# google-research/seed_rl

Hardware: NVIDIA H100
Metric: env-frames/sec (learner, device-timed) on synthetic 84x84x4 T=20 unrolls @1/2/4/8 H100 (higher is better)
Workload: dtype bf16x3 (fp32-faithful tensor-core contraction; activations stored as bf16 hi+lo pairs), f32 elsewhere

## Files before the change

include/seedrl_b200.h:

```cpp
#ifndef SEEDRL_B200_H_
#define SEEDRL_B200_H_

#include <stddef.h>
#include <stdint.h>

#ifdef __cplusplus
extern "C" {
#endif

#define SEEDRL_OK 0
#define SEEDRL_ERR_INVALID_ARGUMENT 3
#define SEEDRL_ERR_OUT_OF_RANGE 11
#define SEEDRL_ERR_INTERNAL 13
#define SEEDRL_ERR_CANCELLED 1
#define SEEDRL_ERR_UNAVAILABLE 14

typedef void* seedrl_stream_t;

const char* seedrl_last_error(void);
int seedrl_abi_version(void);
uint64_t seedrl_kernel_launch_count(void);

int seedrl_vtrace_from_importance_weights(
    int T, int B,
    const float* target_action_log_probs, const float* behaviour_action_log_probs,
    const float* discounts, const float* rewards, const float* values,
    const float* bootstrap_value,
    float clip_rho_threshold, float clip_pg_rho_threshold, float lambda_,
    float* vs, float* pg_advantages, seedrl_stream_t stream);

int seedrl_categorical_log_prob(int N, int A, const float* logits,
                                const int64_t* actions, float* log_prob,
                                seedrl_stream_t stream);
int seedrl_categorical_entropy(int N, int A, const float* logits, float* entropy,
                               seedrl_stream_t stream);
int seedrl_categorical_sample(int N, int A, const float* logits,
                              const float* gumbel_noise, uint64_t seed,
                              uint64_t offset, int64_t* actions,
                              seedrl_stream_t stream);
int seedrl_categorical_sample_counter(int N, int A, const float* logits, const float* gumbel_noise,
                                      uint64_t seed, uint64_t* counter_dev, int64_t* actions,
                                      seedrl_stream_t stream);

typedef struct seedrl_loss_config {
  float discounting;
  float lambda_;
  float baseline_cost;
  float kl_cost;
  float max_abs_reward;
  float clip_rho_threshold;
  float clip_pg_rho_threshold;
  float target_entropy;
  int32_t has_target_entropy;
  float entropy_cost_adjustment_speed;
} seedrl_loss_config;

enum {
  SEEDRL_LT_TOTAL = 0, SEEDRL_LT_POLICY = 1, SEEDRL_LT_V = 2, SEEDRL_LT_ENTROPY = 3,
  SEEDRL_LT_KL = 4, SEEDRL_LT_ENTROPY_ADJ = 5, SEEDRL_LT_V_MEAN = 6,
  SEEDRL_LT_V_L2_ERROR = 7, SEEDRL_LT_MEAN_ENTROPY = 8, SEEDRL_LT_ENTROPY_COST = 9,
  SEEDRL_LT_MEAN_KL = 10, SEEDRL_LT_MAX_ACTION_ABS = 11,
  SEEDRL_LOSS_TERMS = 16
};

size_t seedrl_vtrace_loss_scratch_bytes(int T1, int B, int A);
int seedrl_vtrace_loss_fwd_bwd(
    int T1, int B, int A,
    const float* learner_logits, const float* learner_baseline,
    const float* behaviour_logits, const int64_t* actions,
    const float* rewards, const uint8_t* done,
    const seedrl_loss_config* cfg, const float* entropy_cost_param,
    float* loss_terms, float* dlogits, float* dbaseline,
    float* d_entropy_cost_param, float* vs_out, float* pg_advantages_out,
    void* scratch, seedrl_stream_t stream);

int seedrl_adam_apply(size_t n, float* params, const float* grads, float* m,
                      float* v, float lr_t, float beta1, float beta2, float eps,
                      float grad_scale, int64_t clamp_index, float clamp_lo,
                      float clamp_hi, seedrl_stream_t stream);

enum { SEEDRL_NET_DEEP = 0, SEEDRL_NET_SHALLOW = 1 };

typedef struct seedrl_net_config {
  int32_t net;
  int32_t num_actions;
  int32_t obs_h, obs_w, obs_c;
} seedrl_net_config;

typedef struct seedrl_net seedrl_net;

int seedrl_net_create(const seedrl_net_config* cfg, seedrl_net** out);
void seedrl_net_destroy(seedrl_net* net);
int seedrl_net_num_param_tensors(const seedrl_net* net);
size_t seedrl_net_num_params(const seedrl_net* net);
size_t seedrl_net_arena_floats(const seedrl_net* net);
int seedrl_net_set_conv_mode(seedrl_net* net, int mode);
int seedrl_net_set_lstm_mode(seedrl_net* net, int mode);
int seedrl_net_param_info(const seedrl_net* net, int index, char* name_buf,
                          size_t name_buf_len, int64_t* dims, size_t* offset);
size_t seedrl_net_workspace_bytes(const seedrl_net* net, int T1, int B);

int seedrl_net_forward(const seedrl_net* net, const float* params, int T1, int B,
                       const int64_t* prev_actions, const float* reward,
                       const uint8_t* done, const uint8_t* observation,
                       const float* h0, const float* c0,
                       float* policy_logits, float* baseline,
                       float* h_out, float* c_out,
                       void* workspace, size_t workspace_bytes,
                       seedrl_stream_t stream);
int seedrl_net_backward(const seedrl_net* net, const float* params, int T1, int B,
                        const int64_t* prev_actions, const float* reward,
                        const uint8_t* done, const uint8_t* observation,
                        const float* dlogits, const float* dbaseline,
                        float* grads, void* workspace, size_t workspace_bytes,
                        seedrl_stream_t stream);
int seedrl_net_backward_overlap(const seedrl_net* net, const float* params, int T1, int B,
                                const int64_t* prev_actions, const float* reward, const uint8_t* done,
                                const uint8_t* observation, const float* dlogits, const float* dbaseline,
                                float* grads, void* workspace, size_t workspace_bytes,
                                void* head_ready_event, seedrl_stream_t stream);
size_t seedrl_net_grad_split(const seedrl_net* net);
int seedrl_net_check_error(const seedrl_net* net, int T1, int B, void* workspace,
                           size_t workspace_bytes, seedrl_stream_t stream);

int seedrl_store_append_field(uint8_t* state, const int32_t* index,
                              const int32_t* env_ids, int n, int full_length,
                              size_t row_bytes, const uint8_t* values,
                              seedrl_stream_t stream);
int seedrl_store_advance(int32_t* index, const int32_t* env_ids, int n,
                         int full_length, int32_t* completed_ids,
                         int32_t* num_completed, seedrl_stream_t stream);
int seedrl_store_advance_limit(int32_t* index, const int32_t* env_ids, int n,
                               int full_length, int32_t* completed_ids,
                               int32_t* num_completed, int32_t id_limit,
                               seedrl_stream_t stream);
int seedrl_store_gather_field(uint8_t* state, const int32_t* completed_ids,
                              int n_completed, int full_length, size_t row_bytes,
                              int overlap, int time_major, uint8_t* unrolls,
                              seedrl_stream_t stream);
#define SEEDRL_MAX_ROW_JOBS 16
typedef struct seedrl_row_job {
  void* table;
  void* rows;
  size_t row_bytes;
  int32_t mode;
  int32_t full_length;
} seedrl_row_job;
int seedrl_rows_multi(const seedrl_row_job* jobs, int njobs, const int32_t* env_ids, int n,
                      const int32_t* index, seedrl_stream_t stream);
int seedrl_rows_multi_limit(const seedrl_row_job* jobs, int njobs, const int32_t* env_ids, int n,
                            const int32_t* index, int32_t id_limit, seedrl_stream_t stream);
int seedrl_store_gather_field_into(uint8_t* state, const int32_t* completed_ids, int n_completed,
                                   int full_length, size_t row_bytes, int overlap, uint8_t* batch,
                                   int batch_cols, int col0, seedrl_stream_t stream);
int seedrl_store_finish(int32_t* index, const int32_t* completed_ids,
                        int n_completed, int overlap, seedrl_stream_t stream);
int seedrl_store_reset(uint8_t* state, int32_t* index, const int32_t* env_ids,
                       int n, int full_length, size_t row_bytes, int overlap,
                       seedrl_stream_t stream);

typedef struct seedrl_batcher seedrl_batcher;
int seedrl_batcher_create(int batch_size, int num_slabs, int n_in,
                          const size_t* in_row_bytes, int n_out,
                          const size_t* out_row_bytes, int pinned,
                          seedrl_batcher** out);
void seedrl_batcher_destroy(seedrl_batcher* b);
int seedrl_batcher_claim(seedrl_batcher* b, int k, int* slab, int* row);
void* seedrl_batcher_input_ptr(seedrl_batcher* b, int slab, int field, int row);
void* seedrl_batcher_output_ptr(seedrl_batcher* b, int slab, int field, int row);
int seedrl_batcher_commit(seedrl_batcher* b, int slab, int k);
int seedrl_batcher_wait_outputs(seedrl_batcher* b, int slab, int* status);
int seedrl_batcher_release(seedrl_batcher* b, int slab);
int seedrl_batcher_next_full(seedrl_batcher* b, int timeout_ms, int* slab);
int seedrl_batcher_publish(seedrl_batcher* b, int slab, int status);
int seedrl_batcher_shutdown(seedrl_batcher* b);

int seedrl_profile_num_categories(void);
const char* seedrl_profile_category_name(int i);
int seedrl_profile_begin(seedrl_stream_t stream);
int seedrl_profile_end(double* ms_per_category, uint64_t* launches_per_category);

typedef struct seedrl_r2d2_net seedrl_r2d2_net;
int seedrl_r2d2_net_create(int num_actions, int obs_h, int obs_w, int channels, seedrl_r2d2_net** out);
void seedrl_r2d2_net_destroy(seedrl_r2d2_net* net);
int seedrl_r2d2_net_num_param_tensors(const seedrl_r2d2_net* net);
size_t seedrl_r2d2_net_num_params(const seedrl_r2d2_net* net);
size_t seedrl_r2d2_net_arena_floats(const seedrl_r2d2_net* net);
int seedrl_r2d2_net_set_mode(seedrl_r2d2_net* net, int mode);
int seedrl_r2d2_net_set_lstm_mode(seedrl_r2d2_net* net, int mode);
int seedrl_r2d2_net_param_info(const seedrl_r2d2_net* net, int index, char* name_buf, size_t name_buf_len,
                               int64_t* dims4, int* rank, size_t* offset_floats);
size_t seedrl_r2d2_net_workspace_bytes(const seedrl_r2d2_net* net, int T, int B);
int seedrl_r2d2_net_forward(const seedrl_r2d2_net* net, const float* params, int T, int B,
                            const int64_t* prev_actions, const float* reward, const uint8_t* done,
                            const uint8_t* frames, const float* h0, const float* c0, float* q_values,
                            int32_t* action, float* h_out, float* c_out, void* workspace,
                            size_t workspace_bytes, seedrl_stream_t stream);
int seedrl_r2d2_net_backward(const seedrl_r2d2_net* net, const float* params, int T, int B,
                             const uint8_t* frames, const uint8_t* done, const float* dq, float* grads,
                             void* workspace, size_t workspace_bytes, seedrl_stream_t stream);
int seedrl_r2d2_net_check_error(const seedrl_r2d2_net* net, int T, int B, void* workspace,
                                size_t workspace_bytes, seedrl_stream_t stream);

int seedrl_r2d2_stack_frames(int T, int B, int P, int stack_size, const uint8_t* frames,
                             const int32_t* state_in, const uint8_t* done, uint8_t* stacked,
                             int32_t* state_out, seedrl_stream_t stream);
size_t seedrl_r2d2_loss_scratch_bytes(int T, int B, int n_steps);
int seedrl_r2d2_loss_fwd_bwd(int T, int B, int A, const float* q_train, const float* q_target,
                             const int64_t* replay_action, const float* reward, const uint8_t* done,
                             const float* importance_weights, float gamma, int n_steps, float eta,
                             float value_rescaling_eps, float* loss, float* priorities, float* dq,
                             void* scratch, seedrl_stream_t stream);
int seedrl_r2d2_epsilon_greedy(int N, int A, const int32_t* env_ids, const float* envs_epsilon,
                               uint64_t seed, uint64_t* counter_dev, int32_t* actions,
                               seedrl_stream_t stream);
int seedrl_replay_sample(int limit, const float* priorities, float priority_exp,
                         float importance_sampling_exp, int num_samples, const float* uniforms,
                         int64_t* indices, float* weights, float* probs_out, seedrl_stream_t stream);
size_t seedrl_clip_scratch_bytes(void);
int seedrl_clip_by_global_norm(size_t n, float* grads, float clip_norm, float* norm_out,
                               void* scratch, seedrl_stream_t stream);

int seedrl_debug_conv3x3(int cin, int cout, int in_mode, int N, int H, int W,
                         const void* in, const float* w, const float* bias,
                         const float* mask, const float* res, float* out,
                         seedrl_stream_t stream);
int seedrl_debug_conv3x3_flip(int cin, int cout, const float* w, float* wt,
                              seedrl_stream_t stream);
size_t seedrl_debug_wgrad_partial_bytes(void);
int seedrl_debug_conv_pixels(int N, int H, int W, int which, int start, int count, int* out);
int seedrl_debug_set_loss_stream(int enabled);
int seedrl_debug_set_wgrad_chunk(int kc);
int seedrl_debug_set_conv_tile(int mt);
int seedrl_debug_set_gemm_bk(int bk);
int seedrl_debug_set_gemm_gather(int on);
int seedrl_debug_set_first_layer_dense(int on);
int seedrl_debug_conv0pool(int N, int H, int W, const uint8_t* frames, const float* w, const float* bias,
                           void* praw, void* prelu, uint8_t* idx, int* err, seedrl_stream_t stream);
int seedrl_debug_conv0pool_c(int N, int H, int W, int C, const uint8_t* frames, const float* w, const float* bias,
                             void* praw, void* prelu, uint8_t* idx, int* err, seedrl_stream_t stream);
int seedrl_debug_first_wgrad_pooled_c(int N, int H, int W, int C, const uint8_t* frames, const void* g_planes,
                                      const uint8_t* idx, float* dw, float* db, float* partial,
                                      size_t partial_bytes, seedrl_stream_t stream);
int seedrl_debug_conv3x3_wgrad(int cin, int cout, int in_mode, int N, int H, int W,
                               const void* x, const float* dy, float* dw, float* db,
                               float* partial, size_t partial_bytes,
                               seedrl_stream_t stream);
int seedrl_debug_conv3x3_tc(int cin, int cout, int in_mode, int split, int N, int H, int W,
                            const void* in, const float* w, const float* bias,
                            const float* mask, const float* res, float* out, int flip,
                            int variant, void* wq_scratch, int* error_flag,
                            seedrl_stream_t stream);
int seedrl_debug_conv3x3_wgrad_tc(int cin, int cout, int in_mode, int split, int N, int H, int W,
                                  const void* x, const float* dy, float* dw, float* db,
                                  float* partial, size_t partial_bytes, int* error_flag,
                                  seedrl_stream_t stream);
int seedrl_debug_maxpool(int backward, int N, int H, int W, int C, const float* x_or_dy,
                         float* y_or_dx, uint8_t* idx, seedrl_stream_t stream);
int seedrl_debug_gemm_tc(int ta, int tb, int split, int M, int N, int K, const float* A, int lda,
                         const float* B, int ldb, float* C, int ldc, const float* bias,
                         const float* mask, int ldm, int relu, int accumulate, int a_relu,
                         float* ws, size_t ws_bytes, int* error_flag, seedrl_stream_t stream);
int seedrl_debug_colsum(int M, int N, const float* X, int ld, float* out, float* ws, size_t ws_bytes,
                        seedrl_stream_t stream);
int seedrl_debug_sgemm(int ta, int tb, int M, int N, int K, const float* A, int lda,
                       const float* B, int ldb, float* C, int ldc, const float* bias,
                       const float* mask, int ldm, int relu, int accumulate, int a_relu,
                       seedrl_stream_t stream);
int seedrl_debug_strided_conv(int op, int mode, int gather, int in_u8, int N, int H, int W, int C, int K,
                              int S, int cout, const void* x, const float* w, const float* bias,
                              const float* dy, const float* mask, float* out, int ldo, float* dbias,
                              float* col, size_t col_bytes, float* ws, size_t ws_bytes, int* error_flag,
                              int* gathered, seedrl_stream_t stream);
size_t seedrl_debug_lstm_workspace_bytes(int mode, int H, int T1, int B);
int seedrl_debug_lstm_forward(int mode, int gemm_mode, int H, int T1, int B, const float* U, const uint8_t* done,
                              float* z, const float* h0, const float* c0, float* hs, float* cs, float* hp,
                              void* ws, size_t ws_bytes, int* error_flag, seedrl_stream_t stream);
int seedrl_debug_lstm_backward(int mode, int gemm_mode, int H, int T1, int B, const float* U, const uint8_t* done,
                               const float* gates, const float* cs, const float* c0, const float* dhs, float* dz,
                               void* ws, size_t ws_bytes, int* error_flag, seedrl_stream_t stream);

size_t seedrl_debug_planes_bytes(int N, int H, int W, int C);
int seedrl_debug_to_planes(int N, int H, int W, int C, int relu, const float* x, void* out,
                           seedrl_stream_t stream);
int seedrl_debug_from_planes(int N, int H, int W, int C, const void* in, float* y,
                             seedrl_stream_t stream);
int seedrl_debug_convp(int cin, int cout, int N, int H, int W, const void* in, const float* w,
                       const float* bias, const void* mask, const void* res, int flip,
                       void* out_raw, void* out_relu, float* out_nhwc, void* wq_scratch,
                       int* error_flag, seedrl_stream_t stream);
int seedrl_debug_wgradp(int cin, int cout, int N, int H, int W, const void* x, const void* dy,
                        float* dw, float* db, float* partial, size_t partial_bytes,
                        int* error_flag, seedrl_stream_t stream);
int seedrl_debug_poolp(int backward, int N, int H, int W, int C, const void* in, void* out_raw,
                       void* out_relu, float* out_nhwc, uint8_t* idx, seedrl_stream_t stream);

#ifdef __cplusplus
}
#endif
#endif
```

seed_rl_b200/_lib.py:

```python
import ctypes
import os

_HERE = os.path.dirname(os.path.abspath(__file__))
LIB_PATH = os.path.join(_HERE, 'libseedrl_b200.so')

c_void_p, c_int, c_float, c_size_t = ctypes.c_void_p, ctypes.c_int, ctypes.c_float, ctypes.c_size_t
c_i64, c_u64 = ctypes.c_int64, ctypes.c_uint64
P = c_void_p


class SeedrlError(RuntimeError):

  def __init__(self, code, msg):
    super().__init__('libseedrl_b200 error %d: %s' % (code, msg))
    self.code = code


class LossConfig(ctypes.Structure):
  _fields_ = [('discounting', c_float), ('lambda_', c_float), ('baseline_cost', c_float),
              ('kl_cost', c_float), ('max_abs_reward', c_float),
              ('clip_rho_threshold', c_float), ('clip_pg_rho_threshold', c_float),
              ('target_entropy', c_float), ('has_target_entropy', ctypes.c_int32),
              ('entropy_cost_adjustment_speed', c_float)]


class RowJob(ctypes.Structure):
  _fields_ = [('table', ctypes.c_void_p), ('rows', ctypes.c_void_p), ('row_bytes', ctypes.c_size_t),
              ('mode', ctypes.c_int32), ('full_length', ctypes.c_int32)]


ROW_GATHER, ROW_SCATTER, ROW_APPEND = 0, 1, 2


def rows_multi(jobs, env_ids_i32, index=None, id_limit=None):
  n = int(env_ids_i32.numel())
  arr = (RowJob * len(jobs))()
  for k, (table, rows, mode) in enumerate(jobs):
    rb = (table[0, 0] if mode == ROW_APPEND else table[0]).numel() * table.element_size()
    if rows.numel() * rows.element_size() != n * rb or rows.dtype != table.dtype or not rows.is_contiguous():
      raise ValueError('rows_multi: rows do not match the table (job %d)' % k)
    arr[k] = RowJob(table.data_ptr(), rows.data_ptr(), rb, mode, table.shape[1] if mode == ROW_APPEND else 0)
  if id_limit is None:
    check(lib().seedrl_rows_multi(arr, len(jobs), ptr(env_ids_i32), n, ptr(index), stream_ptr()))
  else:
    check(lib().seedrl_rows_multi_limit(arr, len(jobs), ptr(env_ids_i32), n, ptr(index), int(id_limit),
                                        stream_ptr()))


class NetConfig(ctypes.Structure):
  _fields_ = [('net', ctypes.c_int32), ('num_actions', ctypes.c_int32),
              ('obs_h', ctypes.c_int32), ('obs_w', ctypes.c_int32), ('obs_c', ctypes.c_int32)]


NET_DEEP, NET_SHALLOW = 0, 1
LOSS_TERMS = 16
LT = dict(total=0, policy=1, V=2, entropy=3, kl=4, entropy_adj=5, v_mean=6, v_l2_error=7,
          mean_entropy=8, entropy_cost=9, mean_kl=10, max_action_abs=11)

SIGNATURES = {
    'seedrl_last_error': (ctypes.c_char_p, []),
    'seedrl_abi_version': (c_int, []),
    'seedrl_kernel_launch_count': (c_u64, []),
    'seedrl_vtrace_from_importance_weights':
        (c_int, [c_int, c_int, P, P, P, P, P, P, c_float, c_float, c_float, P, P, P]),
    'seedrl_categorical_log_prob': (c_int, [c_int, c_int, P, P, P, P]),
    'seedrl_categorical_entropy': (c_int, [c_int, c_int, P, P, P]),
    'seedrl_categorical_sample': (c_int, [c_int, c_int, P, P, c_u64, c_u64, P, P]),
    'seedrl_categorical_sample_counter': (c_int, [c_int, c_int, P, P, c_u64, P, P, P]),
    'seedrl_vtrace_loss_scratch_bytes': (c_size_t, [c_int, c_int, c_int]),
    'seedrl_vtrace_loss_fwd_bwd':
        (c_int, [c_int, c_int, c_int, P, P, P, P, P, P, ctypes.POINTER(LossConfig), P,
                 P, P, P, P, P, P, P, P]),
    'seedrl_adam_apply':
        (c_int, [c_size_t, P, P, P, P, c_float, c_float, c_float, c_float, c_float, c_i64,
                 c_float, c_float, P]),
    'seedrl_net_create': (c_int, [ctypes.POINTER(NetConfig), ctypes.POINTER(P)]),
    'seedrl_net_destroy': (None, [P]),
    'seedrl_net_num_param_tensors': (c_int, [P]),
    'seedrl_net_num_params': (c_size_t, [P]),
    'seedrl_net_arena_floats': (c_size_t, [P]),
    'seedrl_net_set_conv_mode': (c_int, [P, c_int]),
    'seedrl_net_set_lstm_mode': (c_int, [P, c_int]),
    'seedrl_net_param_info':
        (c_int, [P, c_int, ctypes.c_char_p, c_size_t, ctypes.POINTER(c_i64),
                 ctypes.POINTER(c_size_t)]),
    'seedrl_net_workspace_bytes': (c_size_t, [P, c_int, c_int]),
    'seedrl_net_forward':
        (c_int, [P, P, c_int, c_int, P, P, P, P, P, P, P, P, P, P, P, c_size_t, P]),
    'seedrl_net_backward':
        (c_int, [P, P, c_int, c_int, P, P, P, P, P, P, P, P, c_size_t, P]),
    'seedrl_net_backward_overlap':
        (c_int, [P, P, c_int, c_int, P, P, P, P, P, P, P, P, c_size_t, P, P]),
    'seedrl_net_grad_split': (c_size_t, [P]),
    'seedrl_net_check_error': (c_int, [P, c_int, c_int, P, c_size_t, P]),
    'seedrl_store_append_field': (c_int, [P, P, P, c_int, c_int, c_size_t, P, P]),
    'seedrl_store_advance': (c_int, [P, P, c_int, c_int, P, P, P]),
    'seedrl_store_advance_limit': (c_int, [P, P, c_int, c_int, P, P, ctypes.c_int32, P]),
    'seedrl_store_gather_field': (c_int, [P, P, c_int, c_int, c_size_t, c_int, c_int, P, P]),
    'seedrl_rows_multi': (c_int, [P, c_int, P, c_int, P, P]),
    'seedrl_rows_multi_limit': (c_int, [P, c_int, P, c_int, P, ctypes.c_int32, P]),
    'seedrl_store_gather_field_into': (c_int, [P, P, c_int, c_int, c_size_t, c_int, P, c_int, c_int, P]),
    'seedrl_store_finish': (c_int, [P, P, c_int, c_int, P]),
    'seedrl_store_reset': (c_int, [P, P, P, c_int, c_int, c_size_t, c_int, P]),
    'seedrl_batcher_create':
        (c_int, [c_int, c_int, c_int, ctypes.POINTER(c_size_t), c_int, ctypes.POINTER(c_size_t),
                 c_int, ctypes.POINTER(P)]),
    'seedrl_batcher_destroy': (None, [P]),
    'seedrl_batcher_claim': (c_int, [P, c_int, ctypes.POINTER(c_int), ctypes.POINTER(c_int)]),
    'seedrl_batcher_input_ptr': (P, [P, c_int, c_int, c_int]),
    'seedrl_batcher_output_ptr': (P, [P, c_int, c_int, c_int]),
    'seedrl_batcher_commit': (c_int, [P, c_int, c_int]),
    'seedrl_batcher_wait_outputs': (c_int, [P, c_int, ctypes.POINTER(c_int)]),
    'seedrl_batcher_release': (c_int, [P, c_int]),
    'seedrl_batcher_next_full': (c_int, [P, c_int, ctypes.POINTER(c_int)]),
    'seedrl_batcher_publish': (c_int, [P, c_int, c_int]),
    'seedrl_batcher_shutdown': (c_int, [P]),
    'seedrl_r2d2_net_create': (c_int, [c_int, c_int, c_int, c_int, ctypes.POINTER(P)]),
    'seedrl_r2d2_net_destroy': (None, [P]),
    'seedrl_r2d2_net_num_param_tensors': (c_int, [P]),
    'seedrl_r2d2_net_num_params': (c_size_t, [P]),
    'seedrl_r2d2_net_arena_floats': (c_size_t, [P]),
    'seedrl_r2d2_net_set_mode': (c_int, [P, c_int]),
    'seedrl_r2d2_net_set_lstm_mode': (c_int, [P, c_int]),
    'seedrl_r2d2_net_param_info':
        (c_int, [P, c_int, ctypes.c_char_p, c_size_t, ctypes.POINTER(c_i64), ctypes.POINTER(c_int),
                 ctypes.POINTER(c_size_t)]),
    'seedrl_r2d2_net_workspace_bytes': (c_size_t, [P, c_int, c_int]),
    'seedrl_r2d2_net_forward':
        (c_int, [P, P, c_int, c_int, P, P, P, P, P, P, P, P, P, P, P, c_size_t, P]),
    'seedrl_r2d2_net_backward': (c_int, [P, P, c_int, c_int, P, P, P, P, P, c_size_t, P]),
    'seedrl_r2d2_net_check_error': (c_int, [P, c_int, c_int, P, c_size_t, P]),
    'seedrl_r2d2_stack_frames': (c_int, [c_int, c_int, c_int, c_int, P, P, P, P, P, P]),
    'seedrl_r2d2_loss_scratch_bytes': (c_size_t, [c_int, c_int, c_int]),
    'seedrl_r2d2_loss_fwd_bwd': (c_int, [c_int, c_int, c_int, P, P, P, P, P, P, c_float, c_int, c_float, c_float,
                                         P, P, P, P, P]),
    'seedrl_r2d2_epsilon_greedy': (c_int, [c_int, c_int, P, P, c_u64, P, P, P]),
    'seedrl_replay_sample': (c_int, [c_int, P, c_float, c_float, c_int, P, P, P, P, P]),
    'seedrl_clip_scratch_bytes': (c_size_t, []),
    'seedrl_clip_by_global_norm': (c_int, [c_size_t, P, c_float, P, P, P]),
    'seedrl_profile_num_categories': (c_int, []),
    'seedrl_profile_category_name': (ctypes.c_char_p, [c_int]),
    'seedrl_profile_begin': (c_int, [P]),
    'seedrl_profile_end': (c_int, [ctypes.POINTER(ctypes.c_double), ctypes.POINTER(c_u64)]),
    'seedrl_debug_planes_bytes': (c_size_t, [c_int, c_int, c_int, c_int]),
    'seedrl_debug_to_planes': (c_int, [c_int, c_int, c_int, c_int, c_int, P, P, P]),
    'seedrl_debug_from_planes': (c_int, [c_int, c_int, c_int, c_int, P, P, P]),
    'seedrl_debug_convp': (c_int, [c_int, c_int, c_int, c_int, c_int, P, P, P, P, P, c_int, P, P, P, P, P, P]),
    'seedrl_debug_wgradp': (c_int, [c_int, c_int, c_int, c_int, c_int, P, P, P, P, P, c_size_t, P, P]),
    'seedrl_debug_poolp': (c_int, [c_int, c_int, c_int, c_int, c_int, P, P, P, P, P, P]),
    'seedrl_debug_conv3x3': (c_int, [c_int, c_int, c_int, c_int, c_int, c_int, P, P, P, P, P, P, P]),
    'seedrl_debug_conv3x3_flip': (c_int, [c_int, c_int, P, P, P]),
    'seedrl_debug_conv3x3_tc':
        (c_int, [c_int, c_int, c_int, c_int, c_int, c_int, c_int, P, P, P, P, P, P, c_int, c_int, P, P, P]),
    'seedrl_debug_wgrad_partial_bytes': (c_size_t, []),
    'seedrl_debug_conv_pixels': (c_int, [c_int, c_int, c_int, c_int, c_int, c_int, P]),
    'seedrl_debug_set_loss_stream': (c_int, [c_int]),
    'seedrl_debug_set_wgrad_chunk': (c_int, [c_int]),
    'seedrl_debug_set_conv_tile': (c_int, [c_int]),
    'seedrl_debug_set_gemm_bk': (c_int, [c_int]),
    'seedrl_debug_set_first_layer_dense': (c_int, [c_int]),
    'seedrl_debug_conv0pool': (c_int, [c_int, c_int, c_int, P, P, P, P, P, P, P, P]),
    'seedrl_debug_conv0pool_c': (c_int, [c_int, c_int, c_int, c_int, P, P, P, P, P, P, P, P]),
    'seedrl_debug_first_wgrad_pooled_c': (c_int, [c_int, c_int, c_int, c_int, P, P, P, P, P, P, c_size_t, P]),
    'seedrl_debug_conv3x3_wgrad_tc':
        (c_int, [c_int, c_int, c_int, c_int, c_int, c_int, c_int, P, P, P, P, P, c_size_t, P, P]),
    'seedrl_debug_conv3x3_wgrad':
        (c_int, [c_int, c_int, c_int, c_int, c_int, c_int, P, P, P, P, P, c_size_t, P]),
    'seedrl_debug_maxpool': (c_int, [c_int, c_int, c_int, c_int, c_int, P, P, P, P]),
    'seedrl_debug_gemm_tc':
        (c_int, [c_int, c_int, c_int, c_int, c_int, c_int, P, c_int, P, c_int, P, c_int, P, P, c_int, c_int, c_int,
                 c_int, P, c_size_t, P, P]),
    'seedrl_debug_set_gemm_gather': (c_int, [c_int]),
    'seedrl_debug_colsum': (c_int, [c_int, c_int, P, c_int, P, P, c_size_t, P]),
    'seedrl_debug_sgemm':
        (c_int, [c_int, c_int, c_int, c_int, c_int, P, c_int, P, c_int, P, c_int, P, P, c_int,
                 c_int, c_int, c_int, P]),
    'seedrl_debug_strided_conv':
        (c_int, [c_int, c_int, c_int, c_int, c_int, c_int, c_int, c_int, c_int, c_int, c_int, P, P, P, P, P, P,
                 c_int, P, P, c_size_t, P, c_size_t, P, ctypes.POINTER(c_int), P]),
    'seedrl_debug_lstm_workspace_bytes': (c_size_t, [c_int, c_int, c_int, c_int]),
    'seedrl_debug_lstm_forward':
        (c_int, [c_int, c_int, c_int, c_int, c_int, P, P, P, P, P, P, P, P, P, c_size_t, P, P]),
    'seedrl_debug_lstm_backward':
        (c_int, [c_int, c_int, c_int, c_int, c_int, P, P, P, P, P, P, P, P, c_size_t, P, P]),
}

_lib = None


def lib():
  global _lib
  if _lib is None:
    if not os.path.exists(LIB_PATH):
      raise ImportError(
          'seed_rl_b200: %s is missing -- build it with `python -c "import '
          '__graft_entry__ as g; g.build()"` (seed_rl_b200/csrc/build.sh). There is no '
          'CPU or PyTorch fallback.' % LIB_PATH)
    l = ctypes.CDLL(LIB_PATH)
    for name, (res, args) in SIGNATURES.items():
      fn = getattr(l, name)
      fn.restype = res
      fn.argtypes = args
    _lib = l
  return _lib


def check(rc):
  if rc != 0:
    raise SeedrlError(rc, (lib().seedrl_last_error() or b'').decode('utf-8', 'replace'))


def launch_count():
  return int(lib().seedrl_kernel_launch_count())


def ptr(t):
  return None if t is None else ctypes.c_void_p(t.data_ptr())


def stream_ptr():
  import torch
  return ctypes.c_void_p(torch.cuda.current_stream().cuda_stream)


def require_cuda(t, dtype, name):
  import torch
  if not isinstance(t, torch.Tensor):
    t = torch.as_tensor(t)
  if not torch.cuda.is_available():
    raise RuntimeError('seed_rl_b200 needs a CUDA device (H100); there is no CPU path '
                       '(argument %r).' % name)
  if t.device.type != 'cuda':
    t = t.cuda()
  if t.dtype != dtype:
    t = t.to(dtype)
  return t.contiguous()
```

seed_rl_b200/common/inference_host.py:

```python
from absl import logging
import numpy as np
import torch

from seed_rl_b200 import _lib
from seed_rl_b200.common import utils
from seed_rl_b200.grpc import ops as grpc


class InferenceHostBase(object):

  algorithm = None

  def __init__(self, agent, num_envs, inference_batch_size, observation_shape, action_dtype,
               agent_state_specs, agent_output_specs, unroll_length, num_overlapping_steps=0,
               time_major=False, id_limit=None, num_action_repeats=1, device='cuda', info_queue=None,
               use_graph=False):
    self.agent = agent
    self.device = torch.device(device)
    self.N = N = int(inference_batch_size)
    self.num_action_repeats = num_action_repeats
    TS = utils.TensorSpec
    self.env_output_specs = utils.EnvOutput(
        TS([], 'float32', 'reward'), TS([], 'bool', 'done'), TS(list(observation_shape), 'uint8', 'observation'),
        TS([], 'bool', 'abandoned'), TS([], 'int32', 'episode_step'))
    action_specs = TS([], action_dtype, 'action')
    self.agent_state_specs = agent_state_specs
    self._id_limit = id_limit
    self._num_store_envs = num_envs if id_limit is None else id_limit
    self.store = utils.UnrollStore(self._num_store_envs, unroll_length,
                                   (action_specs, self.env_output_specs, agent_output_specs),
                                   num_overlapping_steps=num_overlapping_steps, device=device, time_major=time_major)
    self.env_run_ids = np.zeros([num_envs], np.int64)
    self.env_infos = [np.zeros([num_envs], np.int64), np.zeros([num_envs], np.float32),
                      np.zeros([num_envs], np.float32)]
    self.first_agent_states = utils.Aggregator(num_envs, agent_state_specs, 'first_agent_states', device)
    self.agent_states = utils.Aggregator(num_envs, agent_state_specs, 'agent_states', device)
    self.actions = utils.Aggregator(num_envs, action_specs, 'actions', device)
    self.info_queue = info_queue
    self.inference_specs = (
        TS([N], 'int32', 'env_id'), TS([N], 'int64', 'run_id'),
        utils.map_structure(lambda s: TS([N] + list(s.shape), s.dtype, s.name), self.env_output_specs),
        TS([N], 'float32', 'raw_reward'))
    self.output_specs = TS([N], action_dtype, 'action')
    self.stream = torch.cuda.Stream(device=self.device)
    self.use_graph = bool(use_graph)
    if self.use_graph and not 1 <= N <= num_envs:
      raise ValueError('cuda_graph needs 1 <= inference_batch_size <= num_envs, got %d and %d' % (N, num_envs))
    self._graph = None
    self._actions_pin = torch.zeros([N], dtype=utils.as_torch_dtype(action_dtype)).pin_memory()

    @grpc.function(self.inference_specs, self.output_specs)
    def inference(env_ids, run_ids, env_outputs, raw_rewards):
      return self._inference(env_ids, run_ids, env_outputs, raw_rewards)
    self.inference = inference

  def _policy(self, ids32, prev_actions, env_outputs, prev_states, counter):
    raise NotImplementedError

  def _completed_unrolls(self, nc):
    raise NotImplementedError

  def _episode_infos(self, done_ids):
    return tuple(torch.as_tensor(t[done_ids]) for t in self.env_infos)

  def _begin_batch(self, env_ids, run_ids, env_outputs, raw_rewards):
    if np.asarray(env_outputs.abandoned).any():
      raise ValueError('Abandoned done states are not supported in %s.' % self.algorithm)
    utils._check_no_duplicates(None, env_ids, 'inference batch')
    previous = self.env_run_ids[env_ids]
    self.env_run_ids[env_ids] = run_ids
    reset_ids = env_ids[previous != run_ids]
    if reset_ids.size:
      logging.info('Environment ids needing reset: %s', reset_ids)
      for t in self.env_infos:
        t[reset_ids] = 0
      self.store.reset(reset_ids[reset_ids < self._num_store_envs])
      init = self.agent.initial_state(len(reset_ids))
      self.first_agent_states.replace(reset_ids, init)
      self.agent_states.replace(reset_ids, init)
      self.actions.reset(reset_ids)
    self.env_infos[1][env_ids] += np.asarray(env_outputs.reward)
    self.env_infos[2][env_ids] += np.asarray(raw_rewards)
    done_ids = env_ids[np.asarray(env_outputs.done)]
    if self.info_queue is not None and done_ids.size:
      self.info_queue.enqueue_many(self._episode_infos(done_ids))
    for t in self.env_infos:
      t[done_ids] = 0
    self.env_infos[0][env_ids] += self.num_action_repeats

  def _device_step(self, ids32, env_dev, counter):
    n = int(ids32.numel())
    tables = self.agent_states._state
    prev_actions = torch.empty([n], dtype=self.actions._state[0].dtype, device=self.device)
    prev_states = [torch.empty([n] + list(t.shape[1:]), dtype=t.dtype, device=self.device) for t in tables]
    _lib.rows_multi([(self.actions._state[0], prev_actions, _lib.ROW_GATHER)] +
                    [(t, r, _lib.ROW_GATHER) for t, r in zip(tables, prev_states)], ids32)
    agent_outputs, curr_states = self._policy(
        ids32, prev_actions, env_dev, utils.pack_sequence_as(self.agent_state_specs, prev_states), counter)
    self.store.device_append(ids32, utils.flatten((prev_actions, env_dev, agent_outputs)), id_limit=self._id_limit)
    _lib.rows_multi([(t, r.contiguous(), _lib.ROW_SCATTER) for t, r in zip(tables, utils.flatten(curr_states))] +
                    [(self.actions._state[0], agent_outputs.action.contiguous(), _lib.ROW_SCATTER)], ids32)
    return prev_states, agent_outputs

  def _build_graph(self):
    N, dev = self.N, self.device
    self._g_ids = torch.arange(N, dtype=torch.int32, device=dev)
    self._g_env = utils.EnvOutput(*(torch.zeros([N] + list(s.shape), dtype=utils.as_torch_dtype(s.dtype), device=dev)
                                    for s in self.env_output_specs))
    self._g_pin = [torch.zeros_like(t, device='cpu').pin_memory() for t in (self._g_ids,) + tuple(self._g_env)]
    self._g_counter = torch.zeros([], dtype=torch.int64, device=dev)
    touched = (self.actions._state + self.agent_states._state + self.store._state +
               [self.store._index, self._g_counter])
    saved = [t.clone() for t in touched]
    self._device_step(self._g_ids, self._g_env, self._g_counter)
    for t, sv in zip(touched, saved):
      t.copy_(sv)
    self.stream.synchronize()
    g = torch.cuda.CUDAGraph()
    with torch.cuda.graph(g, stream=self.stream, capture_error_mode='thread_local'):
      self._g_prev_states, self._g_out = self._device_step(self._g_ids, self._g_env, self._g_counter)
    self._graph = g

  def _inference(self, env_ids, run_ids, env_outputs, raw_rewards):
    env_ids, run_ids = np.asarray(env_ids), np.asarray(run_ids)
    n = len(env_ids)
    with torch.cuda.stream(self.stream):
      self._begin_batch(env_ids, run_ids, env_outputs, raw_rewards)
      if self.use_graph and n == self.N:
        if self._graph is None:
          self._build_graph()
        srcs = (env_ids.astype(np.int32),) + tuple(np.asarray(x) for x in env_outputs)
        for pin, dst, src in zip(self._g_pin, (self._g_ids,) + tuple(self._g_env), srcs):
          t = torch.from_numpy(np.ascontiguousarray(src))
          if t.numel() >= 65536 and t.is_pinned():
            dst.copy_(t, non_blocking=True)
          else:
            pin.numpy()[...] = src
            dst.copy_(pin, non_blocking=True)
        self._graph.replay()
        prev_states, agent_outputs = self._g_prev_states, self._g_out
      else:
        ids32 = torch.as_tensor(env_ids.astype(np.int32)).to(self.device, non_blocking=True)
        env_dev = utils.EnvOutput(*(torch.as_tensor(np.asarray(x)).to(self.device, non_blocking=True)
                                    for x in env_outputs))
        prev_states, agent_outputs = self._device_step(ids32, env_dev, None)
      store_pos = np.nonzero(env_ids < self._num_store_envs)[0]
      done_ids, pos = self.store.host_advance(env_ids[store_pos])
      pending = None
      if done_ids.size:
        completed_ids, pending = self._completed_unrolls(int(done_ids.size))
        pos_dev = torch.as_tensor(store_pos[pos].astype(np.int64)).to(self.device, non_blocking=True)
        self.first_agent_states.replace(completed_ids, [t.index_select(0, pos_dev) for t in prev_states],
                                        check_unique=False)
      actions = self._actions_pin[:n]
      actions.copy_(agent_outputs.action, non_blocking=True)
      self.stream.synchronize()
    if pending is not None:
      self.unroll_queue.enqueue_many(pending)
    return actions.numpy().copy()
```

seed_rl_b200/csrc/conv_planes.cu:

```cuda
#include <cuda.h>
#include <cuda_bf16.h>

#include <cstdio>
#include <cstdlib>

#include "kernels.h"
#include "tc_common.cuh"

namespace seedrl {

long long planes_positions(int N, int H, int W) {
  const long long Q = (long long)N * (H + 1) * (W + 2);
  return ((Q + 2 * (W + 2) + 2 + 256 + 127) / 128) * 128;
}
size_t planes_bytes(int N, int H, int W, int C) {
  return (size_t)planes_positions(N, H, W) * 16 * 2 * (C / 8);
}

typedef CUresult (*EncodeTiledFn)(CUtensorMap*, CUtensorMapDataType, cuuint32_t, void*, const cuuint64_t*,
                                  const cuuint64_t*, const cuuint32_t*, const cuuint32_t*,
                                  CUtensorMapInterleave, CUtensorMapSwizzle, CUtensorMapL2promotion,
                                  CUtensorMapFloatOOBfill);
static EncodeTiledFn encode_tiled_fn() {
  static EncodeTiledFn fn = nullptr;
  static bool tried = false;
  if (!tried) {
    tried = true;
    void* q = nullptr;
    cudaDriverEntryPointQueryResult qr;
    if (cudaGetDriverEntryPoint("cuTensorMapEncodeTiled", &q, cudaEnableDefault, &qr) == cudaSuccess &&
        qr == cudaDriverEntryPointSuccess)
      fn = reinterpret_cast<EncodeTiledFn>(q);
    (void)cudaGetLastError();
  }
  return fn;
}

static int g_chunk = 0;
int planes_chunk() {
  if (g_chunk == 0) {
    const char* e = getenv("SEEDRL_PLANES_CHUNK");
    g_chunk = e ? atoi(e) : 128;
    if (g_chunk != 16 && g_chunk != 32 && g_chunk != 64 && g_chunk != 128) g_chunk = 128;
  }
  return g_chunk;
}

static int make_plane_map(CUtensorMap* tm, const void* base, long long Lp, int planes, int shift,
                          int CH, int box_chunks, int box_planes) {
  EncodeTiledFn enc = encode_tiled_fn();
  if (!enc) return set_error(SEEDRL_ERR_INTERNAL, "cuTensorMapEncodeTiled is not available");
  if (box_chunks < 1 || box_chunks > 256 || box_planes < 1 || box_planes > planes)
    return set_error(SEEDRL_ERR_INVALID_ARGUMENT, "conv planes: TMA box out of range");
  const cuuint64_t gdim[3] = {(cuuint64_t)(2 * CH), (cuuint64_t)((Lp - shift) / CH), (cuuint64_t)planes};
  const cuuint64_t gstr[2] = {(cuuint64_t)CH * 16, (cuuint64_t)Lp * 16};
  const cuuint32_t box[3] = {(cuuint32_t)(2 * CH), (cuuint32_t)box_chunks, (cuuint32_t)box_planes};
  const cuuint32_t estr[3] = {1, 1, 1};
  void* addr = const_cast<char*>(reinterpret_cast<const char*>(base)) + (size_t)shift * 16;
  const CUresult r = enc(tm, CU_TENSOR_MAP_DATA_TYPE_UINT64, 3, addr, gdim, gstr, box, estr,
                         CU_TENSOR_MAP_INTERLEAVE_NONE, CU_TENSOR_MAP_SWIZZLE_NONE,
                         CU_TENSOR_MAP_L2_PROMOTION_L2_256B, CU_TENSOR_MAP_FLOAT_OOB_FILL_NONE);
  if (r != CUDA_SUCCESS) {
    char msg[128];
    snprintf(msg, sizeof msg, "cuTensorMapEncodeTiled failed (%d) Lp=%lld planes=%d shift=%d box=%dx%d", (int)r, Lp,
             planes, shift, box_chunks, box_planes);
    return set_error(SEEDRL_ERR_INTERNAL, msg);
  }
  return SEEDRL_OK;
}

__device__ __forceinline__ void mbar_expect_tx(uint64_t* bar, uint32_t bytes) {
  asm volatile("mbarrier.arrive.expect_tx.shared::cta.b64 _, [%0], %1;" ::"r"(smem_u32(bar)), "r"(bytes)
               : "memory");
}
__device__ __forceinline__ void tma_load_3d(void* dst, const CUtensorMap* tm, int c0, int c1, int c2,
                                            uint64_t* bar) {
  asm volatile(
      "cp.async.bulk.tensor.3d.shared::cluster.global.tile.mbarrier::complete_tx::bytes [%0], [%1, {%2, %3, %4}], [%5];" ::
          "r"(smem_u32(dst)),
      "l"(reinterpret_cast<uint64_t>(tm)), "r"(c0), "r"(c1), "r"(c2), "r"(smem_u32(bar))
      : "memory");
}
__device__ __forceinline__ float bf16lo(uint32_t w) { return __uint_as_float(w << 16); }
__device__ __forceinline__ float bf16hi(uint32_t w) { return __uint_as_float(w & 0xFFFF0000u); }

struct ConvpArgs {
  ConvGeom g;
  int Lp;
  int nch;
  int chunk;
  int ntiles;
  int nb;
  const uint4* wq;
  const float* bias;
  const uint4* mask;
  const uint4* res;
  uint4* out_raw;
  uint4* out_relu;
  float* out_nhwc;
  int* err;
};

constexpr int kCpWarpgroups = 4;
constexpr int kCpThreads = 128 * kCpWarpgroups + 32;
constexpr int kCpM = 128;
constexpr int kCpMaxStages = 4;

__device__ __forceinline__ void quad_transpose(float2 (&t)[4], int q) {
#pragma unroll
  for (int b = 1; b <= 2; b <<= 1) {
    const bool up = (q & b) != 0;
#pragma unroll
    for (int u = 0; u < 4; ++u) {
      if (u & b) continue;
      const float2 send = up ? t[u] : t[u | b];
      const float2 r = make_float2(__shfl_xor_sync(0xffffffffu, send.x, b), __shfl_xor_sync(0xffffffffu, send.y, b));
      if (up) t[u] = r; else t[u | b] = r;
    }
  }
}

template <int CIN, int COUT, int NSUB>
__global__ void __launch_bounds__(kCpThreads, 1)
convp_kernel(const __grid_constant__ CUtensorMap tm_in, const ConvpArgs a) {
  constexpr int G = CIN / 8, GO = COUT / 8, NS = CIN / 16;
  constexpr int MT = NSUB * kCpM;
  constexpr int NBLK = 2 * NSUB;
  extern __shared__ __align__(128) uint8_t smem_raw[];
  const int PW = a.g.PW, nb = a.nb;
  const uint32_t P = (uint32_t)(a.nch * a.chunk) * 16u;
  const uint32_t stage_bytes = 2u * G * P;
  uint8_t* s_stage = smem_raw;
  uint4* s_b = reinterpret_cast<uint4*>(smem_raw + (size_t)nb * stage_bytes);
  float* s_bias = reinterpret_cast<float*>(s_b + 2 * 9 * CIN * COUT / 8);
  uint64_t* s_full = reinterpret_cast<uint64_t*>(s_bias + COUT);
  uint64_t* s_empty = s_full + kCpMaxStages;
  const int tid = threadIdx.x, warp = tid >> 5, lane = tid & 31;

  for (int i = tid; i < 2 * 9 * CIN * COUT / 8; i += kCpThreads) s_b[i] = __ldg(a.wq + i);
  if (tid < COUT) s_bias[tid] = a.bias ? __ldg(a.bias + tid) : 0.f;
  if (tid == 0) {
    for (int i = 0; i < nb; ++i) {
      mbar_init(s_full + i, 1);
      mbar_init(s_empty + i, 4 * kCpWarpgroups);
    }
    asm volatile("fence.mbarrier_init.release.cluster;" ::: "memory");
    asm volatile("prefetch.tensormap [%0];" ::"l"(reinterpret_cast<uint64_t>(&tm_in)) : "memory");
  }
  asm volatile("fence.proxy.async.shared::cta;" ::: "memory");
  __syncthreads();

  const int my_tiles = ((int)blockIdx.x < a.ntiles) ? (a.ntiles - 1 - (int)blockIdx.x) / (int)gridDim.x + 1 : 0;
  bool timed_out = false;

  if (warp == 4 * kCpWarpgroups) {
    if (elect_one()) {
      for (int it = 0; it < my_tiles; ++it) {
        const int s = it % nb;
        if (it >= nb && !mbar_wait_bounded(s_empty + s, (uint32_t)(((it / nb) - 1) & 1))) { timed_out = true; break; }
        const int tile = (int)blockIdx.x + it * (int)gridDim.x;
        mbar_expect_tx(s_full + s, stage_bytes);
        tma_load_3d(s_stage + (size_t)s * stage_bytes, &tm_in, 0, tile * MT / a.chunk, 0, s_full + s);
      }
    }
    __syncwarp();
  } else {
    const int cw = warp >> 2;
    const size_t plane_u = (size_t)a.Lp;
    if (blockIdx.x == 0) {
      const uint4 z = make_uint4(0u, 0u, 0u, 0u);
      for (int i = tid; i < (PW + 1) * 2 * GO; i += 128 * kCpWarpgroups) {
        const int pl = i / (PW + 1), s = i - pl * (PW + 1);
        if (a.out_raw) a.out_raw[(size_t)pl * plane_u + s] = z;
        if (a.out_relu) a.out_relu[(size_t)pl * plane_u + s] = z;
      }
    }
    const int q = lane & 3;
    const int row = 16 * (warp & 3) + (lane >> 2) + 8 * (q & 1);
    const uint32_t b_base = smem_u32(s_b);
    const uint64_t db0 = gmma_desc(b_base, (uint32_t)(2 * GO) * 128u, 128u);
    for (int it = 0; it < my_tiles; ++it) {
      const int s = it % nb;
      const int tile = (int)blockIdx.x + it * (int)gridDim.x;
      if (!mbar_wait_bounded(s_full + s, (uint32_t)((it / nb) & 1))) { timed_out = true; break; }
      const int m0 = (cw - it * NBLK) & (kCpWarpgroups - 1);
      if (m0 >= NBLK && lane == 0) mbar_arrive(s_empty + s);
      const uint32_t a_base = smem_u32(s_stage + (size_t)s * stage_bytes);
      const uint64_t da0 = gmma_desc(a_base, P, 128u);
      const uint64_t lo_off = (uint64_t)((G * P) >> 4), slab_off = (uint64_t)((2 * P) >> 4);
#pragma unroll 1
      for (int m = m0; m < NBLK; m += kCpWarpgroups) {
        float acc[COUT];
#pragma unroll
        for (int i = 0; i < COUT; ++i) acc[i] = 0.f;
        wgmma_fence_acc<COUT>(acc);
        wgmma_fence();
#pragma unroll
        for (int tap = 0; tap < 9; ++tap) {
          const uint64_t off = (uint64_t)(m * 64 + (tap / 3) * PW + (tap % 3));
#pragma unroll
          for (int sl = 0; sl < NS; ++sl) {
            const uint64_t da = da0 + off + (uint64_t)sl * slab_off;
            const uint64_t db = db0 + (uint64_t)((tap * NS + sl) * (COUT * 64 / 16));
            Wgmma<2 * COUT>::template mma<0, 0>(acc, da, db, 1u);
            Wgmma<COUT>::template mma<0, 0>(acc, da + lo_off, db, 1u);
          }
        }
        wgmma_commit();
        const int p = tile * MT + m * 64 + row;
        const int sp = p + PW + 1;
        const int pix = out_pixel(a.g, p);
        uint4 mk[GO / 2], rh[GO / 2], rl[GO / 2];
        if (pix >= 0) {
#pragma unroll
          for (int k = 0; k < GO / 2; ++k) {
            const int go = (q >> 1) + 2 * k;
            if (a.mask) mk[k] = __ldg(a.mask + (size_t)go * plane_u + sp);
            if (a.res) {
              rh[k] = __ldg(a.res + (size_t)go * plane_u + sp);
              rl[k] = __ldg(a.res + (size_t)(GO + go) * plane_u + sp);
            }
          }
        }
        wgmma_wait<0>();
        wgmma_fence_acc<COUT>(acc);
        if (m + kCpWarpgroups >= NBLK && lane == 0) mbar_arrive(s_empty + s);
        const bool in_store = sp < a.Lp;
#pragma unroll
        for (int k = 0; k < GO / 2; ++k) {
          const int go = (q >> 1) + 2 * k;
          float2 t[4];
#pragma unroll
          for (int u = 0; u < 4; ++u) {
            const int j = 2 * k + (u >> 1), h = u & 1;
            t[u] = make_float2(acc[4 * j + 2 * h] + acc[4 * (j + GO) + 2 * h],
                               acc[4 * j + 2 * h + 1] + acc[4 * (j + GO) + 2 * h + 1]);
          }
          quad_transpose(t, q);
          float x[8];
#pragma unroll
          for (int e = 0; e < 4; ++e) {
            x[2 * e] = t[e].x + s_bias[go * 8 + 2 * e];
            x[2 * e + 1] = t[e].y + s_bias[go * 8 + 2 * e + 1];
          }
          if (pix >= 0 && a.mask) {
            const uint32_t mw[4] = {mk[k].x, mk[k].y, mk[k].z, mk[k].w};
#pragma unroll
            for (int e = 0; e < 4; ++e) {
              x[2 * e] = bf16lo(mw[e]) > 0.f ? x[2 * e] : 0.f;
              x[2 * e + 1] = bf16hi(mw[e]) > 0.f ? x[2 * e + 1] : 0.f;
            }
          }
          if (pix >= 0 && a.res) {
            const uint32_t hw[4] = {rh[k].x, rh[k].y, rh[k].z, rh[k].w};
            const uint32_t lw[4] = {rl[k].x, rl[k].y, rl[k].z, rl[k].w};
#pragma unroll
            for (int e = 0; e < 4; ++e) {
              x[2 * e] += bf16lo(hw[e]) + bf16lo(lw[e]);
              x[2 * e + 1] += bf16hi(hw[e]) + bf16hi(lw[e]);
            }
          }
          if (pix < 0) {
#pragma unroll
            for (int e = 0; e < 8; ++e) x[e] = 0.f;
          }
          const float4 xa = make_float4(x[0], x[1], x[2], x[3]), xb = make_float4(x[4], x[5], x[6], x[7]);
          if (a.out_raw && in_store) {
            a.out_raw[(size_t)go * plane_u + sp] = pack8_bf16(xa, xb);
            a.out_raw[(size_t)(GO + go) * plane_u + sp] = pack8_bf16(bf16_resid4(xa), bf16_resid4(xb));
          }
          if (a.out_relu && in_store) {
            const float4 ra = make_float4(fmaxf(xa.x, 0.f), fmaxf(xa.y, 0.f), fmaxf(xa.z, 0.f), fmaxf(xa.w, 0.f));
            const float4 rb = make_float4(fmaxf(xb.x, 0.f), fmaxf(xb.y, 0.f), fmaxf(xb.z, 0.f), fmaxf(xb.w, 0.f));
            a.out_relu[(size_t)go * plane_u + sp] = pack8_bf16(ra, rb);
            a.out_relu[(size_t)(GO + go) * plane_u + sp] = pack8_bf16(bf16_resid4(ra), bf16_resid4(rb));
          }
          if (a.out_nhwc && pix >= 0) {
            float4* o = reinterpret_cast<float4*>(a.out_nhwc + (size_t)pix * COUT + go * 8);
            o[0] = xa; o[1] = xb;
          }
        }
      }
    }
  }
  if (timed_out && a.err) atomicExch(a.err, 1);
}

template <int CIN, int COUT, int NSUB>
static int launch_convp(const PlaneConv& c, cudaStream_t st) {
  const ConvGeom g = make_geom(c.N, c.H, c.W);
  constexpr int MT = NSUB * kCpM;
  const long long Lp = planes_positions(c.N, c.H, c.W);
  if (Lp + MT + 4 * g.PW >= (1LL << 31))
    return set_error(SEEDRL_ERR_INVALID_ARGUMENT, "convp: batch too large for 32-bit positions");
  const int L = MT + 2 * g.PW + 2;
  const int CH = planes_chunk();
  const int nch = (L + CH - 1) / CH;
  const size_t stage = (size_t)2 * (CIN / 8) * nch * CH * 16;
  const size_t fixed = (size_t)2 * 9 * CIN * COUT * 2 + COUT * 4 + 2 * kCpMaxStages * 8;
  int nb = kCpMaxStages;
  while (nb > 1 && nb * stage + fixed > 227 * 1024) --nb;
  if (nb < 2) return kPlanesTryNext;
  const size_t smem = nb * stage + fixed;
  CUtensorMap tm;
  SEEDRL_TRY(make_plane_map(&tm, c.in, Lp, 2 * (CIN / 8), 0, CH, nch, 2 * (CIN / 8)));
  static bool attr = false;
  if (!attr) {
    SEEDRL_CUDA(cudaFuncSetAttribute(convp_kernel<CIN, COUT, NSUB>, cudaFuncAttributeMaxDynamicSharedMemorySize,
                                     227 * 1024));
    attr = true;
  }
  ConvpArgs a;
  a.g = g; a.Lp = (int)Lp; a.nch = nch; a.chunk = CH; a.nb = nb;
  a.ntiles = (int)((Lp - g.PW - 1 + MT - 1) / MT);
  a.wq = reinterpret_cast<const uint4*>(c.wq); a.bias = c.bias;
  a.mask = reinterpret_cast<const uint4*>(c.mask); a.res = reinterpret_cast<const uint4*>(c.res);
  a.out_raw = reinterpret_cast<uint4*>(c.out_raw); a.out_relu = reinterpret_cast<uint4*>(c.out_relu);
  a.out_nhwc = c.out_nhwc; a.err = c.err;
  const int grid = a.ntiles < kNumSMs ? a.ntiles : kNumSMs;
  convp_kernel<CIN, COUT, NSUB><<<grid, kCpThreads, smem, st>>>(tm, a);
  count_launch(g_conv_cat, st);
  SEEDRL_CHECK_LAUNCH();
  return SEEDRL_OK;
}

bool convp_supported(int cin, int cout) {
  return (cin == 16 || cin == 32) && (cout == 16 || cout == 32);
}

int convp_forward(int cin, int cout, const PlaneConv& c, cudaStream_t st) {
  const long long Lp = planes_positions(c.N, c.H, c.W);
  const bool small = Lp / 512 < 2 * kNumSMs;
#define SEEDRL_CP_CASE(CI, CO_)                                                   \
  if (cin == CI && cout == CO_) {                                                 \
    int rc = kPlanesTryNext;                                                      \
    if (!small) rc = launch_convp<CI, CO_, 4>(c, st);                             \
    if (rc == kPlanesTryNext) rc = launch_convp<CI, CO_, 2>(c, st);               \
    if (rc == kPlanesTryNext) rc = launch_convp<CI, CO_, 1>(c, st);               \
    if (rc == kPlanesTryNext) return set_error(SEEDRL_ERR_INVALID_ARGUMENT, "convp: image too wide"); \
    return rc;                                                                    \
  }
  SEEDRL_CP_CASE(16, 16)
  SEEDRL_CP_CASE(16, 32)
  SEEDRL_CP_CASE(32, 16)
  SEEDRL_CP_CASE(32, 32)
#undef SEEDRL_CP_CASE
  return set_error(SEEDRL_ERR_INVALID_ARGUMENT, "convp: unsupported (cin,cout)");
}

struct WgradpArgs {
  int PW, T, nchunks, nb;
  int chunk;
  float* partial;
  int* err;
};

constexpr int kWpMaxStages = 6;
constexpr int kWpHaloRow = 8;
__host__ __device__ constexpr int wgradp_mtiles(int CP) { return 3 * CP + 1 <= 64 ? 1 : 2; }
__host__ __device__ constexpr int wgradp_khsplit(int CP) { return CP == 16 ? 3 : 1; }
__host__ __device__ constexpr int wgradp_threads(int CP) { return 128 * wgradp_mtiles(CP) * wgradp_khsplit(CP) + 32; }

struct WgradMaps { CUtensorMap x, x_halo, dy, dy_halo; };

template <int CP, int COUT, int KC>
__global__ void __launch_bounds__(wgradp_threads(CP), 1)
wgradp_kernel(const __grid_constant__ WgradMaps tm, const WgradpArgs a) {
  constexpr int G = CP / 8, GO = COUT / 8;
  constexpr int MT = wgradp_mtiles(CP), KSPL = wgradp_khsplit(CP), NCW = MT * KSPL;
  constexpr int NKH = 3 / KSPL;
  constexpr int NW = 9 * CP * COUT + COUT;
  constexpr uint32_t Px = (KC + kWpHaloRow) * 16;
  extern __shared__ __align__(128) uint8_t smem_raw[];
  const int nb = a.nb, PW = a.PW;
  const uint32_t Pd = (uint32_t)(KC + a.T) * 16u;
  const uint32_t x_bytes = 2u * G * Px;
  const uint32_t stage_bytes = x_bytes + 2u * GO * Pd;
  uint64_t* s_full = reinterpret_cast<uint64_t*>(smem_raw);
  uint64_t* s_empty = s_full + kWpMaxStages;
  uint8_t* s_stage = smem_raw + 128;
  const int tid = threadIdx.x, warp = tid >> 5, lane = tid & 31;

  if (tid == 0) {
    for (int i = 0; i < kWpMaxStages; ++i) { mbar_init(s_full + i, 1); mbar_init(s_empty + i, 4 * NCW); }
    asm volatile("fence.mbarrier_init.release.cluster;" ::: "memory");
  }
  __syncthreads();

  const int my_chunks = ((int)blockIdx.x < a.nchunks) ? (a.nchunks - 1 - (int)blockIdx.x) / (int)gridDim.x + 1 : 0;
  bool timed_out = false;

  if (warp == 4 * NCW) {
    if (elect_one()) {
      for (int it = 0; it < my_chunks; ++it) {
        const int s = it % nb;
        if (it >= nb && !mbar_wait_bounded(s_empty + s, (uint32_t)(((it / nb) - 1) & 1))) { timed_out = true; break; }
        const int j0 = ((int)blockIdx.x + it * (int)gridDim.x) * KC;
        uint8_t* xs = s_stage + (size_t)s * stage_bytes;
        uint8_t* ds = xs + x_bytes;
        mbar_expect_tx(s_full + s, stage_bytes);
        for (int p = 0; p < 2 * G; ++p) {
          tma_load_3d(xs + p * Px, &tm.x, 0, j0 / a.chunk, p, s_full + s);
          tma_load_3d(xs + p * Px + KC * 16, &tm.x_halo, 0, (j0 + KC) / kWpHaloRow, p, s_full + s);
        }
        for (int p = 0; p < 2 * GO; ++p) {
          tma_load_3d(ds + p * Pd, &tm.dy, 0, j0 / a.chunk, p, s_full + s);
          tma_load_3d(ds + p * Pd + KC * 16, &tm.dy_halo, 0, (j0 + KC) / kWpHaloRow, p, s_full + s);
        }
      }
    }
    __syncwarp();
  } else {
    const int cw = warp >> 2, mt = cw % MT, kh0 = (cw / MT) * NKH;
    const int mg0 = 8 * mt + 2 * (warp & 3);
    const int mg = mg0 + ((lane >> 3) & 1);
    const uint32_t a_off = (mg < 3 * G ? (uint32_t)(mg % G) * Px + (uint32_t)(mg / G) * 16u : 0u) +
                           (uint32_t)((lane >> 4) * 8 + (lane & 7)) * 16u;
    const bool data0 = mg0 < 3 * G, data1 = mg0 + 1 < 3 * G;
    const uint32_t one = (lane >> 2) == 0 ? 0x3F803F80u : 0u;
    const uint32_t c0 = mg0 == 3 * G ? one : 0u, c1 = mg0 + 1 == 3 * G ? one : 0u;
    float acc[NKH][COUT];
#pragma unroll
    for (int i = 0; i < NKH * COUT; ++i) (&acc[0][0])[i] = 0.f;
    wgmma_fence_acc<NKH * COUT>(&acc[0][0]);
    const uint64_t desc0 = gmma_desc(0u, 128u, Pd);
    const uint32_t desc_lo = (uint32_t)desc0, desc_hi = (uint32_t)(desc0 >> 32);
    for (int it = 0; it < my_chunks; ++it) {
      const int s = it % nb;
      if (!mbar_wait_bounded(s_full + s, (uint32_t)((it / nb) & 1))) { timed_out = true; break; }
      const uint32_t sb = smem_u32(s_stage + (size_t)s * stage_bytes);
      const uint32_t xb = sb + a_off;
      const uint32_t db = desc_lo + ((sb + x_bytes) >> 4) + (uint32_t)((2 - kh0) * PW);
      uint32_t ah[2][4], al[2][4];
#pragma unroll
      for (int ks = 0; ks < KC / 16; ++ks) {
        uint32_t(&h)[4] = ah[ks & 1];
        uint32_t(&l)[4] = al[ks & 1];
        ldsm_x4_trans(h, xb + ks * 256);
        ldsm_x4_trans(l, xb + G * Px + ks * 256);
        if (!data0) { h[0] = h[2] = c0; l[0] = l[2] = 0u; }
        if (!data1) { h[1] = h[3] = c1; l[1] = l[3] = 0u; }
        wgmma_fence();
#pragma unroll
        for (int kh = 0; kh < NKH; ++kh) {
          const uint64_t b = make_desc64(db - (uint32_t)(kh * PW) + (uint32_t)(ks * 16), desc_hi);
          WgmmaRA<2 * COUT>::template mma<1>(acc[kh], h, b, 1u);
          WgmmaRA<COUT>::template mma<1>(acc[kh], l, b, 1u);
        }
        wgmma_commit();
        wgmma_wait<1>();
      }
      wgmma_wait<0>();
      if (lane == 0) mbar_arrive(s_empty + s);
    }
    wgmma_fence_acc<NKH * COUT>(&acc[0][0]);
    float* dst = a.partial + (size_t)blockIdx.x * NW;
#pragma unroll
    for (int h = 0; h < 2; ++h) {
      const int row = 64 * mt + 16 * (warp & 3) + (lane >> 2) + 8 * h;
      const int kw = row / CP, ci = row - kw * CP;
#pragma unroll
      for (int k = 0; k < NKH; ++k) {
        const int kh = kh0 + k;
#pragma unroll
        for (int j = 0; j < GO; ++j) {
#pragma unroll
          for (int e = 0; e < 2; ++e) {
            const int co = 8 * j + 2 * (lane & 3) + e;
            const float v = acc[k][4 * j + 2 * h + e] + acc[k][4 * j + 2 * h + e + COUT / 2];
            if (row < 3 * CP) dst[((size_t)(kh * 3 + kw) * CP + ci) * COUT + co] = v;
            else if (row == 3 * CP && kh == 1) dst[9 * CP * COUT + co] = v;
          }
        }
      }
    }
  }
  if (timed_out && a.err) atomicExch(a.err, 1);
}

template <int CP, int COUT, int KC>
static int launch_wgradp(int N, int H, int W, const void* x, const void* dy, float* dw, float* db, int* err,
                         WgradBatch* batch, cudaStream_t st) {
  const ConvGeom g = make_geom(N, H, W);
  const long long Lp = planes_positions(N, H, W);
  constexpr int G = CP / 8, GO = COUT / 8;
  const int CH = planes_chunk() < KC ? planes_chunk() : KC;
  if (KC % CH) return kPlanesTryNext;
  const int T = (2 * g.PW + kWpHaloRow - 1) / kWpHaloRow * kWpHaloRow;
  const size_t stage = (size_t)2 * G * (KC + kWpHaloRow) * 16 + (size_t)2 * GO * (KC + T) * 16;
  int nb = kWpMaxStages;
  while (nb > 1 && 128 + nb * stage > 227 * 1024) --nb;
  if (nb < 2) return kPlanesTryNext;
  const size_t smem = 128 + nb * stage;
  WgradMaps tm;
  SEEDRL_TRY(make_plane_map(&tm.x, x, Lp, 2 * G, g.PW, CH, KC / CH, 1));
  SEEDRL_TRY(make_plane_map(&tm.x_halo, x, Lp, 2 * G, g.PW, kWpHaloRow, 1, 1));
  SEEDRL_TRY(make_plane_map(&tm.dy, dy, Lp, 2 * GO, 1, CH, KC / CH, 1));
  SEEDRL_TRY(make_plane_map(&tm.dy_halo, dy, Lp, 2 * GO, 1, kWpHaloRow, T / kWpHaloRow, 1));
  static bool attr = false;
  if (!attr) {
    SEEDRL_CUDA(cudaFuncSetAttribute(wgradp_kernel<CP, COUT, KC>, cudaFuncAttributeMaxDynamicSharedMemorySize,
                                     227 * 1024));
    attr = true;
  }
  static const bool dbg = getenv("SEEDRL_DEBUG_LAUNCH") != nullptr;
  if (dbg) fprintf(stderr, "wgradp<%d,%d,%d> CH=%d T=%d nb=%d stage=%zu smem=%zu\n", CP, COUT, KC, CH, T, nb, stage, smem);
  constexpr int NW = 9 * CP * COUT + COUT;
  WgradpArgs a;
  a.PW = g.PW; a.T = T; a.nb = nb; a.err = err; a.chunk = CH;
  a.nchunks = (int)((g.Q + g.PW + KC - 1) / KC);
  const int grid = a.nchunks < kNumSMs ? a.nchunks : kNumSMs;
  if (!batch || batch->n >= kMaxReduceJobs || batch->used + (size_t)grid * NW > batch->cap_floats)
    return set_error(SEEDRL_ERR_INVALID_ARGUMENT, "wgradp: partial buffer too small");
  a.partial = batch->buf + batch->used;
  batch->used += (size_t)grid * NW;
  wgradp_kernel<CP, COUT, KC><<<grid, wgradp_threads(CP), smem, st>>>(tm, a);
  count_launch(PC_CONV_WGRAD, st);
  SEEDRL_CHECK_LAUNCH();
  batch->jobs[batch->n++] = ReduceJob{a.partial, dw, db, grid, 9 * CP * COUT, COUT};
  return SEEDRL_OK;
}

int wgradp(int cin, int cout, int N, int H, int W, const void* x, const void* dy, float* dw, float* db,
           int* err, WgradBatch* batch, cudaStream_t st) {
#define SEEDRL_WP_CASE(CI, CO_, KC0)                                                                        \
  if (cin == CI && cout == CO_) {                                                                           \
    int rc = kPlanesTryNext;                                                                                \
    if constexpr (KC0 >= 256) rc = launch_wgradp<CI, CO_, 256>(N, H, W, x, dy, dw, db, err, batch, st);     \
    if (rc == kPlanesTryNext) rc = launch_wgradp<CI, CO_, 128>(N, H, W, x, dy, dw, db, err, batch, st);     \
    if (rc == kPlanesTryNext) rc = launch_wgradp<CI, CO_, 64>(N, H, W, x, dy, dw, db, err, batch, st);      \
    if (rc == kPlanesTryNext) return set_error(SEEDRL_ERR_INVALID_ARGUMENT, "wgradp: does not fit");        \
    return rc;                                                                                              \
  }
  SEEDRL_WP_CASE(16, 16, 256)
  SEEDRL_WP_CASE(16, 32, 128)
  SEEDRL_WP_CASE(32, 32, 128)
#undef SEEDRL_WP_CASE
  return set_error(SEEDRL_ERR_INVALID_ARGUMENT, "wgradp: unsupported (cin,cout)");
}

__global__ void to_planes_kernel(ConvGeom g, int Lp, int G, int relu, const float* __restrict__ x,
                                 uint4* __restrict__ out) {
  const long long i = (long long)blockIdx.x * blockDim.x + threadIdx.x;
  if (i >= (long long)Lp * G) return;
  const int s = (int)(i / G), go = (int)(i - (long long)s * G);
  const int pix = in_pixel(g, s);
  float4 a = make_float4(0.f, 0.f, 0.f, 0.f), b = a;
  if (pix >= 0) {
    const float4* src = reinterpret_cast<const float4*>(x + (size_t)pix * (G * 8) + go * 8);
    a = __ldg(src); b = __ldg(src + 1);
    if (relu) {
      a.x = fmaxf(a.x, 0.f); a.y = fmaxf(a.y, 0.f); a.z = fmaxf(a.z, 0.f); a.w = fmaxf(a.w, 0.f);
      b.x = fmaxf(b.x, 0.f); b.y = fmaxf(b.y, 0.f); b.z = fmaxf(b.z, 0.f); b.w = fmaxf(b.w, 0.f);
    }
  }
  out[(size_t)go * Lp + s] = pack8_bf16(a, b);
  out[(size_t)(G + go) * Lp + s] = pack8_bf16(bf16_resid4(a), bf16_resid4(b));
}

__global__ void from_planes_kernel(ConvGeom g, int Lp, int G, const uint4* __restrict__ in, float* __restrict__ y) {
  const long long i = (long long)blockIdx.x * blockDim.x + threadIdx.x;
  if (i >= (long long)Lp * G) return;
  const int s = (int)(i / G), go = (int)(i - (long long)s * G);
  const int pix = in_pixel(g, s);
  if (pix < 0) return;
  const uint4 h = __ldg(in + (size_t)go * Lp + s), l = __ldg(in + (size_t)(G + go) * Lp + s);
  float4* dst = reinterpret_cast<float4*>(y + (size_t)pix * (G * 8) + go * 8);
  dst[0] = make_float4(bf16lo(h.x) + bf16lo(l.x), bf16hi(h.x) + bf16hi(l.x), bf16lo(h.y) + bf16lo(l.y),
                       bf16hi(h.y) + bf16hi(l.y));
  dst[1] = make_float4(bf16lo(h.z) + bf16lo(l.z), bf16hi(h.z) + bf16hi(l.z), bf16lo(h.w) + bf16lo(l.w),
                       bf16hi(h.w) + bf16hi(l.w));
}

int to_planes(int N, int H, int W, int C, int relu, const float* x, void* out, cudaStream_t st) {
  const ConvGeom g = make_geom(N, H, W);
  const long long Lp = planes_positions(N, H, W);
  const long long n = Lp * (C / 8);
  to_planes_kernel<<<(unsigned)((n + 255) / 256), 256, 0, st>>>(g, (int)Lp, C / 8, relu, x,
                                                                reinterpret_cast<uint4*>(out));
  count_launch(PC_MISC, st);
  SEEDRL_CHECK_LAUNCH();
  return SEEDRL_OK;
}
int from_planes(int N, int H, int W, int C, const void* in, float* y, cudaStream_t st) {
  const ConvGeom g = make_geom(N, H, W);
  const long long Lp = planes_positions(N, H, W);
  const long long n = Lp * (C / 8);
  from_planes_kernel<<<(unsigned)((n + 255) / 256), 256, 0, st>>>(g, (int)Lp, C / 8,
                                                                  reinterpret_cast<const uint4*>(in), y);
  count_launch(PC_MISC, st);
  SEEDRL_CHECK_LAUNCH();
  return SEEDRL_OK;
}

__global__ void poolp_fwd_kernel(ConvGeom go_, int Lp, int G, int H, int W, int pt, int pl,
                                 const float* __restrict__ x, uint4* __restrict__ out_raw,
                                 uint4* __restrict__ out_relu, uint8_t* __restrict__ idx) {
  const long long i = (long long)blockIdx.x * blockDim.x + threadIdx.x;
  if (i >= (long long)Lp * G) return;
  const int s = (int)(i / G), gq = (int)(i - (long long)s * G);
  const int pix = in_pixel(go_, s);
  float best[8];
  unsigned char arg[8];
#pragma unroll
  for (int e = 0; e < 8; ++e) { best[e] = 0.f; arg[e] = 0; }
  if (pix >= 0) {
    const int Wo = go_.W, Ho = go_.H, C = G * 8;
    const int n = pix / (Ho * Wo), r = pix - n * (Ho * Wo), ho = r / Wo, wo = r - ho * Wo;
#pragma unroll
    for (int e = 0; e < 8; ++e) best[e] = -INFINITY;
#pragma unroll
    for (int kh = 0; kh < 3; ++kh) {
      const int h = ho * 2 - pt + kh;
      if (h < 0 || h >= H) continue;
#pragma unroll
      for (int kw = 0; kw < 3; ++kw) {
        const int w = wo * 2 - pl + kw;
        if (w < 0 || w >= W) continue;
        const float4* src = reinterpret_cast<const float4*>(x + ((size_t)(n * H + h) * W + w) * C + gq * 8);
        const float4 a = __ldg(src), b = __ldg(src + 1);
        const float v[8] = {a.x, a.y, a.z, a.w, b.x, b.y, b.z, b.w};
        const unsigned char t = (unsigned char)(kh * 3 + kw);
#pragma unroll
        for (int e = 0; e < 8; ++e)
          if (v[e] > best[e]) { best[e] = v[e]; arg[e] = t; }
      }
    }
    uint2 packed;
    packed.x = arg[0] | (arg[1] << 8) | (arg[2] << 16) | ((uint32_t)arg[3] << 24);
    packed.y = arg[4] | (arg[5] << 8) | (arg[6] << 16) | ((uint32_t)arg[7] << 24);
    *reinterpret_cast<uint2*>(idx + (size_t)pix * C + gq * 8) = packed;
  }
  const float4 a = make_float4(best[0], best[1], best[2], best[3]), b = make_float4(best[4], best[5], best[6], best[7]);
  out_raw[(size_t)gq * Lp + s] = pack8_bf16(a, b);
  out_raw[(size_t)(G + gq) * Lp + s] = pack8_bf16(bf16_resid4(a), bf16_resid4(b));
  const float4 ra = make_float4(fmaxf(a.x, 0.f), fmaxf(a.y, 0.f), fmaxf(a.z, 0.f), fmaxf(a.w, 0.f));
  const float4 rb = make_float4(fmaxf(b.x, 0.f), fmaxf(b.y, 0.f), fmaxf(b.z, 0.f), fmaxf(b.w, 0.f));
  out_relu[(size_t)gq * Lp + s] = pack8_bf16(ra, rb);
  out_relu[(size_t)(G + gq) * Lp + s] = pack8_bf16(bf16_resid4(ra), bf16_resid4(rb));
}

template <bool OUT_PLANES>
__global__ void poolp_bwd_kernel(ConvGeom gf, int Lpf, ConvGeom gp, int Lpp, int G, int pt, int pl,
                                 const uint4* __restrict__ dy, const uint8_t* __restrict__ idx,
                                 uint4* __restrict__ dx_planes, float* __restrict__ dx_nhwc) {
  const long long i = (long long)blockIdx.x * blockDim.x + threadIdx.x;
  const int H = gf.H, W = gf.W, Ho = gp.H, Wo = gp.W, C = G * 8;
  int gq, s = 0, pix;
  if (OUT_PLANES) {
    if (i >= (long long)Lpf * G) return;
    s = (int)(i / G); gq = (int)(i - (long long)s * G);
    pix = in_pixel(gf, s);
  } else {
    if (i >= (long long)gf.N * H * W * G) return;
    pix = (int)(i / G); gq = (int)(i - (long long)pix * G);
  }
  float acc[8];
#pragma unroll
  for (int e = 0; e < 8; ++e) acc[e] = 0.f;
  if (pix >= 0) {
    const int n = pix / (H * W), r = pix - n * (H * W), h = r / W, w = r - h * W;
    const int hp = h + pt, wp = w + pl;
#pragma unroll
    for (int dh = 0; dh < 2; ++dh) {
      const int ho = (hp >> 1) - dh;
      const int kh = hp - 2 * ho;
      if (ho < 0 || ho >= Ho || kh > 2) continue;
#pragma unroll
      for (int dw = 0; dw < 2; ++dw) {
        const int wo = (wp >> 1) - dw;
        const int kw = wp - 2 * wo;
        if (wo < 0 || wo >= Wo || kw > 2) continue;
        const unsigned tap = (unsigned)(kh * 3 + kw);
        const size_t o = ((size_t)(n * Ho + ho) * Wo + wo) * C + gq * 8;
        const uint2 t = __ldg(reinterpret_cast<const uint2*>(idx + o));
        const int sp = (n * gp.RH + ho + 1) * gp.PW + wo + 1;
        const uint4 hh = __ldg(dy + (size_t)gq * Lpp + sp), ll = __ldg(dy + (size_t)(G + gq) * Lpp + sp);
        const float gv[8] = {bf16lo(hh.x) + bf16lo(ll.x), bf16hi(hh.x) + bf16hi(ll.x), bf16lo(hh.y) + bf16lo(ll.y),
                             bf16hi(hh.y) + bf16hi(ll.y), bf16lo(hh.z) + bf16lo(ll.z), bf16hi(hh.z) + bf16hi(ll.z),
                             bf16lo(hh.w) + bf16lo(ll.w), bf16hi(hh.w) + bf16hi(ll.w)};
#pragma unroll
        for (int e = 0; e < 8; ++e) {
          const unsigned te = ((e < 4 ? t.x : t.y) >> (8 * (e & 3))) & 0xFFu;
          if (te == tap) acc[e] += gv[e];
        }
      }
    }
  }
  const float4 a = make_float4(acc[0], acc[1], acc[2], acc[3]), b = make_float4(acc[4], acc[5], acc[6], acc[7]);
  if (OUT_PLANES) {
    dx_planes[(size_t)gq * Lpf + s] = pack8_bf16(a, b);
    dx_planes[(size_t)(G + gq) * Lpf + s] = pack8_bf16(bf16_resid4(a), bf16_resid4(b));
  } else {
    float4* dst = reinterpret_cast<float4*>(dx_nhwc + (size_t)pix * C + gq * 8);
    dst[0] = a; dst[1] = b;
  }
}

static void same_pad3s2(int in, int* out, int* before) {
  *out = (in + 1) / 2;
  const int total = (*out - 1) * 2 + 3 - in;
  *before = total > 0 ? total / 2 : 0;
}

int poolp_forward(int N, int H, int W, int C, const float* x, void* out_raw, void* out_relu, uint8_t* idx,
                  cudaStream_t st) {
  int Ho, Wo, pt, pl;
  same_pad3s2(H, &Ho, &pt);
  same_pad3s2(W, &Wo, &pl);
  const ConvGeom g = make_geom(N, Ho, Wo);
  const long long Lp = planes_positions(N, Ho, Wo);
  const long long n = Lp * (C / 8);
  poolp_fwd_kernel<<<(unsigned)((n + 255) / 256), 256, 0, st>>>(g, (int)Lp, C / 8, H, W, pt, pl, x,
                                                                reinterpret_cast<uint4*>(out_raw),
                                                                reinterpret_cast<uint4*>(out_relu), idx);
  count_launch(PC_POOL, st);
  SEEDRL_CHECK_LAUNCH();
  return SEEDRL_OK;
}

int poolp_backward(int N, int H, int W, int C, const void* dy, const uint8_t* idx, void* dx_planes,
                   float* dx_nhwc, cudaStream_t st) {
  int Ho, Wo, pt, pl;
  same_pad3s2(H, &Ho, &pt);
  same_pad3s2(W, &Wo, &pl);
  const ConvGeom gf = make_geom(N, H, W), gp = make_geom(N, Ho, Wo);
  const long long Lpf = planes_positions(N, H, W), Lpp = planes_positions(N, Ho, Wo);
  if (dx_planes) {
    const long long n = Lpf * (C / 8);
    poolp_bwd_kernel<true><<<(unsigned)((n + 255) / 256), 256, 0, st>>>(
        gf, (int)Lpf, gp, (int)Lpp, C / 8, pt, pl, reinterpret_cast<const uint4*>(dy), idx,
        reinterpret_cast<uint4*>(dx_planes), nullptr);
  } else {
    const long long n = (long long)N * H * W * (C / 8);
    poolp_bwd_kernel<false><<<(unsigned)((n + 255) / 256), 256, 0, st>>>(
        gf, (int)Lpf, gp, (int)Lpp, C / 8, pt, pl, reinterpret_cast<const uint4*>(dy), idx, nullptr, dx_nhwc);
  }
  count_launch(PC_POOL, st);
  SEEDRL_CHECK_LAUNCH();
  return SEEDRL_OK;
}

}
```

seed_rl_b200/csrc/kernels.h:

```cpp
#pragma once
#include "common.cuh"

namespace seedrl {

enum { IN_F32 = 0, IN_RELU = 1, IN_U8 = 2 };

struct ConvGeom {
  int N, H, W;
  int PW;
  int RH;
  long long Q;
  unsigned int pw_mul, rh_mul;
  int pw_sh, rh_sh;
};

__host__ __device__ inline void fast_div_setup(unsigned int d, unsigned int* mul, int* sh) {
  int l = 1;
  while ((1u << l) < d) ++l;
  *mul = (unsigned int)(((1ULL << (31 + l)) + d - 1) / d);
  *sh = l - 1;
}
__host__ __device__ __forceinline__ unsigned int fast_div(unsigned int n, unsigned int mul, int sh) {
#ifdef __CUDA_ARCH__
  return __umulhi(n, mul) >> sh;
#else
  return (unsigned int)(((unsigned long long)n * mul) >> 32) >> sh;
#endif
}

__host__ __device__ inline ConvGeom make_geom(int N, int H, int W) {
  ConvGeom g;
  g.N = N; g.H = H; g.W = W; g.PW = W + 2; g.RH = H + 1;
  g.Q = (long long)N * g.RH * g.PW;
  fast_div_setup((unsigned int)g.PW, &g.pw_mul, &g.pw_sh);
  fast_div_setup((unsigned int)g.RH, &g.rh_mul, &g.rh_sh);
  return g;
}

__host__ __device__ __forceinline__ int in_pixel(const ConvGeom& g, int gp) {
  const int Rp = (int)fast_div((unsigned int)gp, g.pw_mul, g.pw_sh);
  const int c = gp - Rp * g.PW;
  const int n = (int)fast_div((unsigned int)Rp, g.rh_mul, g.rh_sh);
  const int rr = Rp - n * g.RH;
  if (rr == 0 || c == 0 || c > g.W || n >= g.N) return -1;
  return (n * g.H + (rr - 1)) * g.W + (c - 1);
}
__host__ __device__ __forceinline__ int out_pixel(const ConvGeom& g, int p) {
  const int Ro = (int)fast_div((unsigned int)p, g.pw_mul, g.pw_sh);
  const int c = p - Ro * g.PW;
  const int n = (int)fast_div((unsigned int)Ro, g.rh_mul, g.rh_sh);
  const int h = Ro - n * g.RH;
  if (h >= g.H || c >= g.W || n >= g.N) return -1;
  return (n * g.H + h) * g.W + c;
}

constexpr int kMaxPackJobs = 32, kMaxReduceJobs = 16;
struct PackJob { const float* w; void* wq; int ck, cout, cin_src, flip, legacy; };
struct PackTable { PackJob jobs[kMaxPackJobs]; int n; };
struct ReduceJob { const float* partial; float* dw; float* db; int nparts, nw, nb; };
struct ReduceTable { ReduceJob jobs[kMaxReduceJobs]; };
struct WgradBatch { float* buf; size_t cap_floats, used; int n; ReduceJob jobs[kMaxReduceJobs]; };

bool conv3x3_tc_supported(int cin, int cout, int in_mode);
int conv3x3_tc_pack_weights(int cin, int cout, int flip, int split, const float* w, void* wq,
                            cudaStream_t st);
bool conv3x3_wgrad_tc_supported(int cin, int cout, int in_mode);
void conv3x3_wgrad_tc_set_chunk(int kc);
int conv3x3_wgrad_tc(int cin, int cout, int in_mode, int split, int N, int H, int W, const void* x,
                     const float* dy, float* dw, float* db, float* partial, size_t partial_bytes,
                     int* err, WgradBatch* batch, cudaStream_t st);
int wgrad_reduce_batch(WgradBatch* b, cudaStream_t st);
int conv3x3_tc_pack_weights_batch(const PackTable& t, int split, cudaStream_t st);
void conv3x3_tc_set_tile(int mt);
int conv3x3_tc_forward(int cin, int cout, int in_mode, int split, int N, int H, int W, const void* in,
                       const void* wq, const float* bias, const float* mask, const float* res,
                       float* out, int variant, int* err, cudaStream_t st);

constexpr int kPlanesTryNext = -12347;
long long planes_positions(int N, int H, int W);
size_t planes_bytes(int N, int H, int W, int C);
struct PlaneConv {
  int N, H, W;
  const void* in;
  const void* wq;
  const float* bias;
  const void* mask;
  const void* res;
  void* out_raw;
  void* out_relu;
  float* out_nhwc;
  int* err;
};
bool convp_supported(int cin, int cout);
int convp_forward(int cin, int cout, const PlaneConv& c, cudaStream_t st);
int wgradp(int cin, int cout, int N, int H, int W, const void* x, const void* dy, float* dw, float* db,
           int* err, WgradBatch* batch, cudaStream_t st);
int to_planes(int N, int H, int W, int C, int relu, const float* x, void* out, cudaStream_t st);
int from_planes(int N, int H, int W, int C, const void* in, float* y, cudaStream_t st);
int poolp_forward(int N, int H, int W, int C, const float* x, void* out_raw, void* out_relu, uint8_t* idx,
                  cudaStream_t st);
int poolp_backward(int N, int H, int W, int C, const void* dy, const uint8_t* idx, void* dx_planes,
                   float* dx_nhwc, cudaStream_t st);

bool first_wgrad_pooled_supported(int cin, int cout, int H, int W);
int first_wgrad_pooled(int N, int H, int W, int C, const uint8_t* frames, const void* g_planes, const uint8_t* idx,
                       float* dw, float* db, WgradBatch* batch, cudaStream_t st);
bool conv0pool_supported(int cin, int cout, int H, int W);
int conv0pool_forward(int N, int H, int W, int C, const uint8_t* frames, const float* w, const float* bias,
                      void* praw, void* prelu, uint8_t* idx, int* err, cudaStream_t st);

int conv3x3_forward(int cin, int cout, int in_mode, int N, int H, int W, const void* in,
                    const float* w, const float* bias, const float* mask, const float* res,
                    float* out, cudaStream_t st);
int conv3x3_u8_forward(int C, int N, int H, int W, const uint8_t* frames, const float* w, const float* bias,
                       float* out, cudaStream_t st);
int conv3x3_u8_wgrad(int C, int N, int H, int W, const uint8_t* frames, const float* dy, float* dw, float* db,
                     float* partial, size_t partial_bytes, cudaStream_t st);
int conv3x3_flip_weights(int cin, int cout, const float* w, float* wt, cudaStream_t st);
size_t conv3x3_wgrad_partial_bytes();
int wgrad_reduce(int nparts, int nw, int nb, const float* partial, float* dw, float* db,
                 cudaStream_t st);
int conv3x3_wgrad(int cin, int cout, int in_mode, int N, int H, int W, const void* x,
                  const float* dy, float* dw, float* db, float* partial, size_t partial_bytes,
                  cudaStream_t st);
int maxpool3s2_forward(int N, int H, int W, int C, const float* x, float* y, uint8_t* idx,
                       cudaStream_t st);
int maxpool3s2_backward(int N, int H, int W, int C, const float* dy, const uint8_t* idx, float* dx,
                        cudaStream_t st);

int convgen_forward(int N, int H, int W, int cin, int cout, int k, int stride, int in_u8,
                    const void* in, const float* w, const float* bias, int relu, float* out,
                    cudaStream_t st);
int convgen_dgrad(int N, int H, int W, int cin, int cout, int k, int stride, const float* dy,
                  const float* w, const float* mask, float* dx, cudaStream_t st);
int convgen_wgrad(int N, int H, int W, int cin, int cout, int k, int stride, int in_u8,
                  const void* x, const float* dy, float* dw, float* db, float* partial,
                  size_t partial_bytes, cudaStream_t st);


struct GemmEpi {
  const float* bias;
  const float* mask;
  int ldm;
  int relu;
  int accumulate;
  int a_relu;
};
inline GemmEpi epi_none() { return GemmEpi{nullptr, nullptr, 0, 0, 0, 0}; }
int sgemm(bool ta, bool tb, int M, int N, int K, const float* A, int lda, const float* B, int ldb,
          float* C, int ldc, const GemmEpi& e, cudaStream_t st);
int colsum(int M, int N, const float* X, int ld, float* out, cudaStream_t st, float* ws = nullptr,
           size_t ws_bytes = 0);
bool gemm_tc_supported(int M, int N, int K);
void gemm_tc_set_bk(int bk);
size_t gemm_tc_workspace_bytes();
struct ConvGather {
  const void* x;
  int u8;
  int H, W, C, S, Ho, Wo;
  int KC;
  unsigned int wo_mul, ho_mul, kc_mul;
  int wo_sh, ho_sh, kc_sh;
};
bool conv_gather_setup(const void* x, int u8, int N, int H, int W, int C, int K, int S, ConvGather* g);
void gemm_tc_set_gather(int on);
bool gemm_tc_gather_enabled();
int gemm_tc(bool ta, bool tb, int split, int M, int N, int K, const float* A, int lda, const float* B,
            int ldb, float* C, int ldc, const GemmEpi& e, float* ws, size_t ws_bytes, int* err,
            cudaStream_t st, const ConvGather* cg = nullptr);
int core_input_tail(int Nrows, int D, int A, const float* reward, const int64_t* prev_action,
                    float* core_in, cudaStream_t st);
int lstm_mask_state(int B, int Hd, const uint8_t* done, const float* h_src, float* h_dst,
                    cudaStream_t st);
int lstm_pointwise_fwd(int B, int Hd, float* z, const float* c_prev_src, const uint8_t* done_t,
                       const uint8_t* done_next, float* c_out, float* h_out, float* hprev_next,
                       cudaStream_t st);
int lstm_pointwise_bwd(int B, int Hd, const float* gates, const float* c_t, const float* c_prev_src,
                       const uint8_t* done_t, const uint8_t* done_next, const float* dh_out,
                       const float* dh_rec, const float* dc_next, float* dz, float* dc_prev_out,
                       cudaStream_t st);
int fill(size_t n, float* p, float v, cudaStream_t st);

int lstm_forward_persistent(int H, int T1, int B, const float* U, const uint8_t* done, float* z,
                            const float* h0, const float* c0, float* hs, float* cs, float* hp,
                            unsigned int* counter, int* err, cudaStream_t st);
int lstm_backward_persistent(int H, int T1, int B, const float* U, const uint8_t* done, const float* gates,
                             const float* cs, const float* c0, const float* dhs, float* dz,
                             unsigned int* counter, int* err, cudaStream_t st);

int lstm_forward_tiled(int H, int T1, int B, const float* U, const uint8_t* done, float* z, const float* h0,
                       const float* c0, float* hs, float* cs, float* hp, unsigned int* counter, int* err,
                       cudaStream_t st);
int lstm_backward_tiled(int H, int T1, int B, const float* U, const uint8_t* done, const float* gates,
                        const float* cs, const float* c0, const float* dhs, float* dz, unsigned int* counter,
                        int* err, cudaStream_t st);

int lstm_forward_tc(int H, int T1, int B, const float* U, const uint8_t* done, float* z, const float* h0,
                    const float* c0, float* hs, float* cs, float* hp, unsigned int* counter, int* err,
                    cudaStream_t st);
int lstm_backward_tc(int H, int T1, int B, const float* U, const uint8_t* done, const float* gates,
                     const float* cs, const float* c0, const float* dhs, float* dz, unsigned int* counter,
                     int* err, cudaStream_t st);

}
```

seed_rl_b200/csrc/net.cu:

```cuda
#include "schedule.h"

namespace seedrl {

constexpr int kHidden = 256;

struct ConvLayer {
  int cin, cout;
  int w, b;
};
struct Stack {
  int hin, win, cin, c, hout, wout;
  ConvLayer conv, r00, r01, r10, r11;
};

}

struct seedrl_net {
  seedrl_net_config cfg;
  seedrl::ParamTable params;
  size_t logical_params;
  int p_base_w, p_base_b, p_dense_w, p_dense_b, p_core_w, p_core_u, p_core_b, p_pol_w, p_pol_b;
  std::vector<seedrl::Stack> stacks;
  seedrl::StridedConv sh[2];
  int sh_w[2], sh_b[2];
  int flat;
  int lstm_mode = 2;
  int conv_mode = 0;
  int core_in;
};

namespace seedrl {

static ConvLayer add_conv(seedrl_net* n, const std::string& prefix, int k, int cin, int cout) {
  ConvLayer l;
  l.cin = cin; l.cout = cout;
  l.w = n->params.add(prefix + "/kernel", {k, k, cin, cout});
  l.b = n->params.add(prefix + "/bias", {cout});
  return l;
}

struct StackBufs {
  size_t a0, p, idx, c0, o0, c1, o1;
  size_t praw, prelu, c0r, o0raw, o0relu, c1r, o1p;
};

constexpr size_t kPackSlotBytes = 2 * 9 * 32 * 32 * 2;
constexpr size_t kPartialAllBytes = (size_t)64 << 20;

struct Plan {
  int N;
  std::vector<StackBufs> st;
  size_t sh_a1, sh_a2;
  size_t sh_col0, sh_col1;
  size_t xc, z, hp, cs, hs, c0buf;
  size_t dhs, dz, dhrec, dc0, dc1, dd, gA, gB, gC, gFull, wt, partial, wq, tcerr, counter, gemm_ws, wq_all, partial_all;
  size_t gP1, gP2, gP3, gFP;
  size_t obs4, w0pad, dw0pad;
  size_t total;
};

static Plan make_plan(const seedrl_net* n, int T1, int B) {
  Plan p;
  Bump b;
  const size_t N = (size_t)T1 * B;
  p.N = (int)N;
  size_t pooled_max = 0, full_max = 0, pooled_planes_max = 0, full_planes_max = 0;
  const bool planes = n->conv_mode == 3 && n->cfg.net == SEEDRL_NET_DEEP;
  if (n->cfg.net == SEEDRL_NET_DEEP) {
    for (size_t si = 0; si < n->stacks.size(); ++si) {
      const Stack& s = n->stacks[si];
      StackBufs sb = StackBufs();
      const size_t full = N * s.hin * s.win * s.c, pooled = N * s.hout * s.wout * s.c;
      sb.a0 = b.take(full * 4);
      sb.idx = b.take(pooled);
      if (!planes) {
        sb.p = b.take(pooled * 4);
        sb.c0 = b.take(pooled * 4);
        sb.o0 = b.take(pooled * 4);
        sb.c1 = b.take(pooled * 4);
        sb.o1 = b.take(pooled * 4);
      } else {
        const size_t pb = planes_bytes((int)N, s.hout, s.wout, s.c);
        sb.praw = b.take(pb); sb.prelu = b.take(pb); sb.c0r = b.take(pb);
        sb.o0raw = b.take(pb); sb.o0relu = b.take(pb); sb.c1r = b.take(pb);
        if (si + 1 < n->stacks.size()) sb.o1p = b.take(pb); else sb.o1 = b.take(pooled * 4);
        if (pb > pooled_planes_max) pooled_planes_max = pb;
        if (si > 0) {
          const size_t fb = planes_bytes((int)N, s.hin, s.win, s.c);
          if (fb > full_planes_max) full_planes_max = fb;
        }
      }
      p.st.push_back(sb);
      if (pooled > pooled_max) pooled_max = pooled;
      if (full > full_max) full_max = full;
    }
    p.sh_a1 = p.sh_a2 = 0;
  } else {
    const StridedConv &l0 = n->sh[0], &l1 = n->sh[1];
    const size_t a1 = N * l0.hout * l0.wout * l0.cout, a2 = N * l1.hout * l1.wout * l1.cout;
    p.sh_a1 = b.take(a1 * 4);
    p.sh_a2 = b.take(a2 * 4);
    p.sh_col0 = p.sh_col1 = 0;
    if (n->conv_mode >= 1) {
      p.sh_col0 = b.take(N * l0.hout * l0.wout * (size_t)(l0.k * l0.k * l0.cin) * 4);
      p.sh_col1 = b.take(N * l1.hout * l1.wout * (size_t)(l1.k * l1.k * l1.cin) * 4);
    }
    pooled_max = a1 > a2 ? a1 : a2;
    full_max = 0;
  }
  p.xc = b.take(N * n->core_in * 4);
  p.z = b.take(N * 4 * kHidden * 4);
  p.hp = b.take(N * kHidden * 4);
  p.cs = b.take(N * kHidden * 4);
  p.hs = b.take(N * kHidden * 4);
  p.c0buf = b.take((size_t)B * kHidden * 4);
  p.dhs = b.take(N * kHidden * 4);
  p.dz = b.take(N * 4 * kHidden * 4);
  p.dhrec = b.take((size_t)B * kHidden * 4);
  p.dc0 = b.take((size_t)B * kHidden * 4);
  p.dc1 = b.take((size_t)B * kHidden * 4);
  p.dd = b.take(N * kHidden * 4);
  p.obs4 = p.w0pad = p.dw0pad = 0;
  if (n->cfg.net == SEEDRL_NET_DEEP && n->cfg.obs_c == 3) {
    p.obs4 = b.take(N * n->cfg.obs_h * n->cfg.obs_w * 4);
    p.w0pad = b.take(9 * 4 * 16 * 4);
    p.dw0pad = b.take(9 * 4 * 16 * 4);
  }
  p.gA = b.take(pooled_max * 4);
  p.gB = p.gC = p.gP1 = p.gP2 = p.gP3 = p.gFP = 0;
  if (!planes) {
    p.gB = b.take(pooled_max * 4);
    p.gC = b.take(pooled_max * 4);
  } else {
    p.gP1 = b.take(pooled_planes_max);
    p.gP2 = b.take(pooled_planes_max);
    p.gP3 = b.take(pooled_planes_max);
    p.gFP = b.take(full_planes_max);
  }
  p.gFull = b.take(full_max * 4);
  p.wt = b.take(64 * 1024 * 4);
  p.wq = b.take(2 * 64 * 1024 * 2);
  p.gemm_ws = b.take(gemm_tc_workspace_bytes());
  p.wq_all = b.take((size_t)kMaxPackJobs * kPackSlotBytes);
  p.partial_all = b.take(kPartialAllBytes);
  p.tcerr = b.take(256);
  p.counter = b.take(256);
  p.partial = b.take(conv3x3_wgrad_partial_bytes());
  p.total = b.off;
  return p;
}

struct Call {
  const seedrl_net* n;
  const Plan& pl;
  const float* prm;
  float* grd;
  void* ws;
  GemmExec ex;
  PackTable packed;
  WgradBatch wb;
  cudaEvent_t head_ready = nullptr;
  int w0_index = -1;
  const float* w0_pad = nullptr;
  float* dw0_pad = nullptr;

  Call(const seedrl_net* n_, const Plan& pl_, const float* prm_, float* grd_, void* ws_, cudaStream_t st)
      : n(n_), pl(pl_), prm(prm_), grd(grd_), ws(ws_),
        ex{n_->conv_mode >= 2 ? 2 : n_->conv_mode, gemm_tc_gather_enabled(), W<float>(ws_, pl_.gemm_ws),
           gemm_tc_workspace_bytes(), W<int>(ws_, pl_.tcerr), st},
        wb{nullptr, 0, 0, 0, {}} {
    packed.n = 0;
  }
  const float* P(int idx) const { return idx == w0_index && w0_pad ? w0_pad : prm + n->params.offset(idx); }
  float* G(int idx) const { return idx == w0_index && dw0_pad ? dw0_pad : grd + n->params.offset(idx); }
};

__global__ void pad_frames3_kernel(size_t npix, const uint8_t* __restrict__ src, uchar4* __restrict__ dst) {
  const size_t i = (size_t)blockIdx.x * blockDim.x + threadIdx.x;
  if (i >= npix) return;
  dst[i] = make_uchar4(src[3 * i], src[3 * i + 1], src[3 * i + 2], 0);
}
__global__ void pad_w0_kernel(int cout, const float* __restrict__ w, float* __restrict__ wp) {
  const int i = blockIdx.x * blockDim.x + threadIdx.x;
  if (i >= 9 * 4 * cout) return;
  const int co = i % cout, ci = (i / cout) % 4, tap = i / (4 * cout);
  wp[i] = ci < 3 ? w[(tap * 3 + ci) * cout + co] : 0.f;
}
__global__ void unpad_dw0_kernel(int cout, const float* __restrict__ dwp, float* __restrict__ dw) {
  const int i = blockIdx.x * blockDim.x + threadIdx.x;
  if (i >= 9 * 3 * cout) return;
  const int co = i % cout, ci = (i / cout) % 3, tap = i / (3 * cout);
  dw[i] = dwp[(tap * 4 + ci) * cout + co];
}

static int g_first_dense = 0;

static inline int first_c(const seedrl_net* n) { return n->cfg.obs_c == 3 ? 4 : n->cfg.obs_c; }
static inline bool generic_first(const seedrl_net* n) {
  return n->cfg.net == SEEDRL_NET_DEEP && first_c(n) != 4;
}

static int pack_all_weights(Call& c, int flip) {
  const seedrl_net* n = c.n;
  c.packed.n = 0;
  if (n->conv_mode < 1 || n->cfg.net != SEEDRL_NET_DEEP) return SEEDRL_OK;
  char* base = W<char>(c.ws, c.pl.wq_all);
  for (size_t s = 0; s < n->stacks.size(); ++s) {
    const Stack& k = n->stacks[s];
    const ConvLayer* ls[5] = {&k.conv, &k.r00, &k.r01, &k.r10, &k.r11};
    for (int i = 0; i < 5; ++i) {
      const ConvLayer& l = *ls[i];
      if (flip && s == 0 && i == 0) continue;
      if (s == 0 && i == 0 && generic_first(n)) continue;
      const int cin = flip ? l.cout : l.cin, cout = flip ? l.cin : l.cout;
      if (c.packed.n >= kMaxPackJobs) return SEEDRL_OK;
      PackJob j;
      j.w = c.P(l.w);
      j.wq = base + (size_t)c.packed.n * kPackSlotBytes;
      j.ck = cin < 16 ? 16 : cin; j.cout = cout; j.cin_src = cin; j.flip = flip;
      j.legacy = (s == 0 && i == 0) ? 1 : 0;
      c.packed.jobs[c.packed.n++] = j;
    }
  }
  return conv3x3_tc_pack_weights_batch(c.packed, n->conv_mode == 3 ? 2 : (n->conv_mode >= 2 ? 1 : 0), c.ex.st);
}
static int packed_weights(const Call& c, int cin, int cout, const float* w, int flip, int split, const void** wq) {
  for (int i = 0; i < c.packed.n; ++i)
    if (c.packed.jobs[i].w == w && c.packed.jobs[i].flip == flip) {
      *wq = c.packed.jobs[i].wq;
      return SEEDRL_OK;
    }
  void* scratch = W<void>(c.ws, c.pl.wq);
  SEEDRL_TRY(conv3x3_tc_pack_weights(cin, cout, flip, split, w, scratch, c.ex.st));
  *wq = scratch;
  return SEEDRL_OK;
}

static int run_conv(const Call& c, int cin, int cout, int in_mode, int N, int H, int Wd, const void* in,
                    const float* w, const float* bias, const float* mask, const float* res, float* out, int flip) {
  cudaStream_t st = c.ex.st;
  if (c.n->conv_mode >= 1 && conv3x3_tc_supported(cin, cout, in_mode)) {
    const int split = c.n->conv_mode >= 2;
    const void* wq;
    SEEDRL_TRY(packed_weights(c, cin, cout, w, flip, split, &wq));
    return conv3x3_tc_forward(cin, cout, in_mode, split, N, H, Wd, in, wq, bias, mask, res, out, 0, c.ex.err, st);
  }
  if (flip) {
    float* wt = W<float>(c.ws, c.pl.wt);
    SEEDRL_TRY(conv3x3_flip_weights(cout, cin, w, wt, st));
    return conv3x3_forward(cin, cout, in_mode, N, H, Wd, in, wt, bias, mask, res, out, st);
  }
  return conv3x3_forward(cin, cout, in_mode, N, H, Wd, in, w, bias, mask, res, out, st);
}

static int pad_first_layer(Call& c, const uint8_t** obs) {
  const seedrl_net* n = c.n;
  if (n->cfg.net != SEEDRL_NET_DEEP || n->cfg.obs_c != 3) return SEEDRL_OK;
  const Plan& pl = c.pl;
  cudaStream_t st = c.ex.st;
  const size_t npix = (size_t)pl.N * n->cfg.obs_h * n->cfg.obs_w;
  pad_frames3_kernel<<<(unsigned)((npix + 255) / 256), 256, 0, st>>>(npix, *obs, W<uchar4>(c.ws, pl.obs4));
  count_launch(PC_MISC, st);
  const int wi = n->stacks[0].conv.w;
  pad_w0_kernel<<<ceil_div(9 * 4 * 16, 128), 128, 0, st>>>(16, c.prm + n->params.offset(wi), W<float>(c.ws, pl.w0pad));
  count_launch(PC_MISC, st);
  if (cudaGetLastError() != cudaSuccess) return set_error(SEEDRL_ERR_INTERNAL, "3-channel padding launch failed");
  *obs = W<uint8_t>(c.ws, pl.obs4);
  c.w0_index = wi; c.w0_pad = W<float>(c.ws, pl.w0pad); c.dw0_pad = W<float>(c.ws, pl.dw0pad);
  return SEEDRL_OK;
}

}

using namespace seedrl;

extern "C" int seedrl_net_create(const seedrl_net_config* cfg, seedrl_net** out) {
  SEEDRL_CHECK_ARG(cfg && out, "null pointer");
  SEEDRL_CHECK_ARG(cfg->net == SEEDRL_NET_DEEP || cfg->net == SEEDRL_NET_SHALLOW, "unknown net");
  SEEDRL_CHECK_ARG(cfg->num_actions >= 1 && cfg->obs_h > 0 && cfg->obs_w > 0, "bad shape");
  seedrl_net* n = new seedrl_net();
  n->cfg = *cfg;
  const int A = cfg->num_actions;
  n->core_in = kHidden + 1 + A;
  n->p_base_w = n->params.add("baseline/kernel", {kHidden, 1});
  n->p_base_b = n->params.add("baseline/bias", {1});
  int flat = 0;
  if (cfg->net == SEEDRL_NET_DEEP) {
    if (cfg->obs_c < 1 || cfg->obs_c > 16) {
      delete n;
      return set_error(SEEDRL_ERR_INVALID_ARGUMENT,
                       "seedrl_net_create: the deep net takes uint8 frames with 1 to 16 channels");
    }
    int h = cfg->obs_h, w = cfg->obs_w;
    const int chans[3] = {16, 32, 32};
    for (int s = 0; s < 3; ++s) { h = (h + 1) / 2; w = (w + 1) / 2; }
    flat = h * w * chans[2];
  } else {
    n->sh[0] = StridedConv(8, 4, cfg->obs_c, 16, cfg->obs_h, cfg->obs_w);
    n->sh[1] = StridedConv(4, 2, 16, 32, n->sh[0].hout, n->sh[0].wout);
    flat = n->sh[1].hout * n->sh[1].wout * 32;
  }
  n->flat = flat;
  n->p_dense_w = n->params.add("conv_to_linear/kernel", {flat, kHidden});
  n->p_dense_b = n->params.add("conv_to_linear/bias", {kHidden});
  n->p_core_w = n->params.add("core/kernel", {n->core_in, 4 * kHidden});
  n->p_core_u = n->params.add("core/recurrent_kernel", {kHidden, 4 * kHidden});
  n->p_core_b = n->params.add("core/bias", {4 * kHidden});
  n->p_pol_w = n->params.add("policy_logits/kernel", {kHidden, A});
  n->p_pol_b = n->params.add("policy_logits/bias", {A});
  if (cfg->net == SEEDRL_NET_DEEP) {
    int h = cfg->obs_h, w = cfg->obs_w, c = cfg->obs_c;
    const int chans[3] = {16, 32, 32};
    for (int s = 0; s < 3; ++s) {
      Stack st;
      const std::string pre = "stack" + std::to_string(s);
      st.hin = h; st.win = w; st.cin = s == 0 ? (c <= 4 ? 4 : (c <= 8 ? 8 : 16)) : c; st.c = chans[s];
      st.hout = (h + 1) / 2; st.wout = (w + 1) / 2;
      st.conv = add_conv(n, pre + "/conv", 3, c, st.c);
      st.conv.cin = st.cin;
      st.r00 = add_conv(n, pre + "/res_0/conv2d_0", 3, st.c, st.c);
      st.r10 = add_conv(n, pre + "/res_1/conv2d_0", 3, st.c, st.c);
      st.r01 = add_conv(n, pre + "/res_0/conv2d_1", 3, st.c, st.c);
      st.r11 = add_conv(n, pre + "/res_1/conv2d_1", 3, st.c, st.c);
      n->stacks.push_back(st);
      h = st.hout; w = st.wout; c = st.c;
    }
  } else {
    for (int i = 0; i < 2; ++i) {
      const StridedConv& l = n->sh[i];
      const ConvLayer cl = add_conv(n, "conv" + std::to_string(i), l.k, l.cin, l.cout);
      n->sh_w[i] = cl.w; n->sh_b[i] = cl.b;
    }
  }
  n->logical_params = 0;
  for (const ParamInfo& p : n->params.list) n->logical_params += p.size;
  n->params.add("entropy_cost_param", {});
  *out = n;
  return SEEDRL_OK;
}

extern "C" void seedrl_net_destroy(seedrl_net* net) { delete net; }
extern "C" int seedrl_net_num_param_tensors(const seedrl_net* net) {
  return net ? (int)net->params.list.size() - 1 : 0;
}
extern "C" size_t seedrl_net_num_params(const seedrl_net* net) { return net ? net->logical_params : 0; }
extern "C" size_t seedrl_net_arena_floats(const seedrl_net* net) { return net ? net->params.arena_floats : 0; }
extern "C" int seedrl_net_set_lstm_mode(seedrl_net* net, int mode) {
  SEEDRL_CHECK_ARG(net && mode >= 0 && mode <= 3, "mode must be 0 (per-step launches), 1 (persistent, CTA = 2 units), 2 (persistent, CTA = batch tile x 16 units) or 3 (as 2 on wgmma bf16x3)");
  net->lstm_mode = mode;
  return SEEDRL_OK;
}
extern "C" int seedrl_net_set_conv_mode(seedrl_net* net, int mode) {
  SEEDRL_CHECK_ARG(net && mode >= 0 && mode <= 3,
                   "mode must be 0 (fp32 SIMT), 1 (wgmma bf16), 2 (wgmma bf16x3) or 3 (bf16x3 plane tensors)");
  SEEDRL_CHECK_ARG(mode != 3 || net->cfg.net == SEEDRL_NET_DEEP, "mode 3 is built for the deep net");
  SEEDRL_CHECK_ARG(!generic_first(net) || (mode != 1 && mode != 2),
                   "conv modes 1 (tc) and 2 (tc3) take 3- or 4-channel frames in the deep net; use 0 (simt) or 3 (tc3p)");
  SEEDRL_CHECK_ARG(!generic_first(net) || mode != 3 ||
                       conv0pool_supported(first_c(net), 16, net->cfg.obs_h, net->cfg.obs_w),
                   "conv mode 3 (tc3p) takes frames of 3 to 107 pixels per side for this channel count; use 0 (simt)");
  net->conv_mode = mode;
  return SEEDRL_OK;
}

extern "C" int seedrl_net_param_info(const seedrl_net* net, int index, char* name_buf,
                                     size_t name_buf_len, int64_t* dims, size_t* offset) {
  const ParamInfo* p = net ? net->params.info(index, name_buf, name_buf_len, dims, offset) : nullptr;
  return p ? p->rank : -1;
}

extern "C" size_t seedrl_net_workspace_bytes(const seedrl_net* net, int T1, int B) {
  if (!net || T1 <= 0 || B <= 0) return 0;
  return make_plan(net, T1, B).total;
}

static int torso_forward_deep(const Call& c, const uint8_t* obs) {
  const seedrl_net* n = c.n; const Plan& pl = c.pl; void* ws = c.ws; cudaStream_t st = c.ex.st;
  const int N = pl.N;
  const void* in = obs;
  int in_mode = IN_U8;
  for (size_t s = 0; s < n->stacks.size(); ++s) {
    const Stack& k = n->stacks[s];
    const StackBufs& b = pl.st[s];
    float* a0 = W<float>(ws, b.a0); float* p = W<float>(ws, b.p);
    float* c0 = W<float>(ws, b.c0); float* o0 = W<float>(ws, b.o0);
    float* c1 = W<float>(ws, b.c1); float* o1 = W<float>(ws, b.o1);
    if (s == 0 && generic_first(n))
      SEEDRL_TRY(conv3x3_u8_forward(first_c(n), N, k.hin, k.win, obs, c.P(k.conv.w), c.P(k.conv.b), a0,
                                    st));
    else
      SEEDRL_TRY(run_conv(c, k.cin, k.c, in_mode, N, k.hin, k.win, in, c.P(k.conv.w),
                          c.P(k.conv.b), nullptr, nullptr, a0, 0));
    SEEDRL_TRY(maxpool3s2_forward(N, k.hin, k.win, k.c, a0, p, W<uint8_t>(ws, b.idx), st));
    SEEDRL_TRY(run_conv(c, k.c, k.c, IN_RELU, N, k.hout, k.wout, p, c.P(k.r00.w),
                        c.P(k.r00.b), nullptr, nullptr, c0, 0));
    SEEDRL_TRY(run_conv(c, k.c, k.c, IN_RELU, N, k.hout, k.wout, c0, c.P(k.r01.w),
                        c.P(k.r01.b), nullptr, p, o0, 0));
    SEEDRL_TRY(run_conv(c, k.c, k.c, IN_RELU, N, k.hout, k.wout, o0, c.P(k.r10.w),
                        c.P(k.r10.b), nullptr, nullptr, c1, 0));
    SEEDRL_TRY(run_conv(c, k.c, k.c, IN_RELU, N, k.hout, k.wout, c1, c.P(k.r11.w),
                        c.P(k.r11.b), nullptr, o0, o1, 0));
    in = o1;
    in_mode = IN_F32;
  }
  return SEEDRL_OK;
}

static int planes_conv(const Call& c, int cin, int cout, int N, int H, int Wd, const void* in, const float* w,
                       int flip, const float* bias, const void* mask, const void* res, void* out_raw, void* out_relu,
                       float* out_nhwc) {
  const void* wq;
  SEEDRL_TRY(packed_weights(c, cin, cout, w, flip, 2, &wq));
  PlaneConv pc;
  pc.N = N; pc.H = H; pc.W = Wd; pc.in = in; pc.wq = wq; pc.bias = bias; pc.mask = mask; pc.res = res;
  pc.out_raw = out_raw; pc.out_relu = out_relu; pc.out_nhwc = out_nhwc; pc.err = c.ex.err;
  return convp_forward(cin, cout, pc, c.ex.st);
}

static int torso_forward_planes(const Call& c, const uint8_t* obs) {
  const seedrl_net* n = c.n; const Plan& pl = c.pl; void* ws = c.ws; cudaStream_t st = c.ex.st;
  const int N = pl.N;
  const void* prev = nullptr;
  const size_t ns = n->stacks.size();
  for (size_t s = 0; s < ns; ++s) {
    const Stack& k = n->stacks[s];
    const StackBufs& b = pl.st[s];
    float* a0 = W<float>(ws, b.a0);
    void* praw = W<void>(ws, b.praw); void* prelu = W<void>(ws, b.prelu);
    void* c0r = W<void>(ws, b.c0r); void* o0raw = W<void>(ws, b.o0raw);
    void* o0relu = W<void>(ws, b.o0relu); void* c1r = W<void>(ws, b.c1r);
    const bool last = s + 1 == ns;
    if (s == 0 && generic_first(n) && g_first_dense)
      return set_error(SEEDRL_ERR_INVALID_ARGUMENT,
                       "the dense first-layer path takes 3- or 4-channel frames; switch it off for these frames");
    if (s == 0 && conv0pool_supported(first_c(n), k.c, k.hin, k.win) && !g_first_dense) {
      SEEDRL_TRY(conv0pool_forward(N, k.hin, k.win, first_c(n), obs, c.P(k.conv.w), c.P(k.conv.b), praw,
                                   prelu, W<uint8_t>(ws, b.idx), W<int>(ws, pl.tcerr), st));
    } else if (s == 0 && generic_first(n)) {
      return set_error(SEEDRL_ERR_INVALID_ARGUMENT, "conv mode 3: the fused first layer takes frames up to 107 pixels wide");
    } else {
      if (s == 0)
        SEEDRL_TRY(run_conv(c, k.cin, k.c, IN_U8, N, k.hin, k.win, obs, c.P(k.conv.w),
                            c.P(k.conv.b), nullptr, nullptr, a0, 0));
      else
        SEEDRL_TRY(planes_conv(c, k.cin, k.c, N, k.hin, k.win, prev, c.P(k.conv.w), 0,
                               c.P(k.conv.b), nullptr, nullptr, nullptr, nullptr, a0));
      SEEDRL_TRY(poolp_forward(N, k.hin, k.win, k.c, a0, praw, prelu, W<uint8_t>(ws, b.idx), st));
    }
    const int H = k.hout, Wd = k.wout, C = k.c;
    SEEDRL_TRY(planes_conv(c, C, C, N, H, Wd, prelu, c.P(k.r00.w), 0, c.P(k.r00.b), nullptr,
                           nullptr, nullptr, c0r, nullptr));
    SEEDRL_TRY(planes_conv(c, C, C, N, H, Wd, c0r, c.P(k.r01.w), 0, c.P(k.r01.b), nullptr,
                           praw, o0raw, o0relu, nullptr));
    SEEDRL_TRY(planes_conv(c, C, C, N, H, Wd, o0relu, c.P(k.r10.w), 0, c.P(k.r10.b), nullptr,
                           nullptr, nullptr, c1r, nullptr));
    SEEDRL_TRY(planes_conv(c, C, C, N, H, Wd, c1r, c.P(k.r11.w), 0, c.P(k.r11.b), nullptr,
                           o0raw, last ? nullptr : W<void>(ws, b.o1p), nullptr,
                           last ? W<float>(ws, b.o1) : nullptr));
    prev = W<void>(ws, b.o1p);
  }
  return SEEDRL_OK;
}

static int torso_forward_shallow(const Call& c, const uint8_t* obs) {
  const seedrl_net* n = c.n; const Plan& pl = c.pl; void* ws = c.ws; cudaStream_t st = c.ex.st;
  const int N = pl.N;
  float* a1 = W<float>(ws, pl.sh_a1);
  float* a2 = W<float>(ws, pl.sh_a2);
  if (n->conv_mode >= 1 && n->cfg.obs_c % 4 == 0) {
    SEEDRL_TRY(n->sh[0].forward(c.ex, N, true, obs, c.P(n->sh_w[0]), c.P(n->sh_b[0]), W<float>(ws, pl.sh_col0), a1,
                                16));
    return n->sh[1].forward(c.ex, N, false, a1, c.P(n->sh_w[1]), c.P(n->sh_b[1]), W<float>(ws, pl.sh_col1), a2, 32);
  }
  SEEDRL_TRY(convgen_forward(N, n->cfg.obs_h, n->cfg.obs_w, n->cfg.obs_c, 16, 8, 4, 1, obs,
                             c.P(n->sh_w[0]), c.P(n->sh_b[0]), 1, a1, st));
  SEEDRL_TRY(convgen_forward(N, n->sh[0].hout, n->sh[0].wout, 16, 32, 4, 2, 0, a1, c.P(n->sh_w[1]),
                             c.P(n->sh_b[1]), 1, a2, st));
  return SEEDRL_OK;
}

extern "C" int seedrl_net_forward(const seedrl_net* n, const float* prm, int T1, int B,
                                  const int64_t* prev_actions, const float* reward,
                                  const uint8_t* done, const uint8_t* observation,
                                  const float* h0, const float* c0, float* policy_logits,
                                  float* baseline, float* h_out, float* c_out, void* ws,
                                  size_t ws_bytes, seedrl_stream_t stream) {
  SEEDRL_CHECK_ARG(n && prm && prev_actions && reward && done && observation && h0 && c0 &&
                       policy_logits && baseline && ws, "null pointer");
  SEEDRL_CHECK_ARG(T1 >= 1 && B >= 1, "T1, B must be >= 1");
  const Plan pl = make_plan(n, T1, B);
  SEEDRL_CHECK_ARG(ws_bytes >= pl.total, "workspace too small");
  cudaStream_t st = (cudaStream_t)stream;
  Call c(n, pl, prm, nullptr, ws, st);
  const int N = pl.N, A = n->cfg.num_actions, CI = n->core_in;
  SEEDRL_CUDA(cudaMemsetAsync(W<int>(ws, pl.tcerr), 0, sizeof(int), st));
  const float* flat_src;
  int flat_relu;
  if (n->cfg.net == SEEDRL_NET_DEEP) {
    SEEDRL_TRY(pad_first_layer(c, &observation));
    SEEDRL_TRY(pack_all_weights(c, 0));
    SEEDRL_TRY(n->conv_mode == 3 ? torso_forward_planes(c, observation) : torso_forward_deep(c, observation));
    flat_src = W<float>(ws, pl.st.back().o1);
    flat_relu = 1;
  } else {
    SEEDRL_TRY(torso_forward_shallow(c, observation));
    flat_src = W<float>(ws, pl.sh_a2);
    flat_relu = 0;
  }
  float* xc = W<float>(ws, pl.xc);
  float* z = W<float>(ws, pl.z);
  float* hp = W<float>(ws, pl.hp);
  float* cs = W<float>(ws, pl.cs);
  float* hs = W<float>(ws, pl.hs);
  float* c0buf = W<float>(ws, pl.c0buf);
  GemmEpi e = epi_none();
  e.bias = c.P(n->p_dense_b); e.relu = 1; e.a_relu = flat_relu;
  SEEDRL_TRY(c.ex.gemm(false, false, N, kHidden, n->flat, flat_src, n->flat, c.P(n->p_dense_w),
                   kHidden, xc, CI, e));
  SEEDRL_TRY(core_input_tail(N, kHidden, A, reward, prev_actions, xc, st));
  e = epi_none();
  e.bias = c.P(n->p_core_b);
  SEEDRL_TRY(c.ex.gemm(false, false, N, 4 * kHidden, CI, xc, CI, c.P(n->p_core_w), 4 * kHidden, z,
                   4 * kHidden, e));
  SEEDRL_CUDA(cudaMemcpyAsync(c0buf, c0, (size_t)B * kHidden * 4, cudaMemcpyDeviceToDevice, st));
  SEEDRL_TRY(lstm_recurrence_forward(n->lstm_mode, c.ex, kHidden, T1, B, c.P(n->p_core_u), done, z, h0, c0buf, hs,
                                     cs, hp, W<unsigned int>(ws, pl.counter)));
  e = epi_none();
  e.bias = c.P(n->p_pol_b);
  SEEDRL_TRY(c.ex.gemm(false, false, N, A, kHidden, hs, kHidden, c.P(n->p_pol_w), A, policy_logits,
                   A, e));
  e.bias = c.P(n->p_base_b);
  SEEDRL_TRY(c.ex.gemm(false, false, N, 1, kHidden, hs, kHidden, c.P(n->p_base_w), 1, baseline, 1,
                   e));
  if (h_out)
    SEEDRL_CUDA(cudaMemcpyAsync(h_out, hs + (size_t)(T1 - 1) * B * kHidden, (size_t)B * kHidden * 4,
                                cudaMemcpyDeviceToDevice, st));
  if (c_out)
    SEEDRL_CUDA(cudaMemcpyAsync(c_out, cs + (size_t)(T1 - 1) * B * kHidden, (size_t)B * kHidden * 4,
                                cudaMemcpyDeviceToDevice, st));
  return SEEDRL_OK;
}

extern "C" int seedrl_net_check_error(const seedrl_net* n, int T1, int B, void* ws, size_t ws_bytes,
                                      seedrl_stream_t stream) {
  SEEDRL_CHECK_ARG(n && ws && T1 >= 1 && B >= 1, "bad arguments");
  const Plan pl = make_plan(n, T1, B);
  SEEDRL_CHECK_ARG(ws_bytes >= pl.total, "workspace too small");
  return read_error_flag(W<int>(ws, pl.tcerr), (cudaStream_t)stream, "step");
}

static int conv_bwd(Call& c, const ConvLayer& l, int N, int H, int Wd, const void* x, int x_mode, const float* dy,
                    const float* dmask, const float* dres, float* dx) {
  const seedrl_net* n = c.n; const Plan& pl = c.pl; void* ws = c.ws; cudaStream_t st = c.ex.st;
  if (n->conv_mode >= 1 && conv3x3_wgrad_tc_supported(l.cin, l.cout, x_mode)) {
    SEEDRL_TRY(conv3x3_wgrad_tc(l.cin, l.cout, x_mode, n->conv_mode >= 2, N, H, Wd, x, dy,
                                c.G(l.w), c.G(l.b), W<float>(ws, pl.partial),
                                conv3x3_wgrad_partial_bytes(), c.ex.err, &c.wb, st));
  } else {
    SEEDRL_TRY(conv3x3_wgrad(l.cin, l.cout, x_mode, N, H, Wd, x, dy, c.G(l.w), c.G(l.b),
                             W<float>(ws, pl.partial), conv3x3_wgrad_partial_bytes(), st));
  }
  if (dx) {
    g_conv_cat = PC_CONV_DGRAD;
    const int rc = run_conv(c, l.cout, l.cin, IN_F32, N, H, Wd, dy, c.P(l.w), nullptr,
                            dmask, dres, dx, 1);
    g_conv_cat = PC_CONV_FWD;
    SEEDRL_TRY(rc);
  }
  return SEEDRL_OK;
}

static int torso_backward_deep(Call& c, const uint8_t* obs) {
  const seedrl_net* n = c.n; const Plan& pl = c.pl; void* ws = c.ws; cudaStream_t st = c.ex.st;
  const int N = pl.N;
  float* gA = W<float>(ws, pl.gA); float* gB = W<float>(ws, pl.gB);
  float* gC = W<float>(ws, pl.gC); float* gF = W<float>(ws, pl.gFull);
  for (int s = (int)n->stacks.size() - 1; s >= 0; --s) {
    const Stack& k = n->stacks[s];
    const StackBufs& b = pl.st[s];
    const float* p = W<float>(ws, b.p);  const float* c0 = W<float>(ws, b.c0);
    const float* o0 = W<float>(ws, b.o0); const float* c1 = W<float>(ws, b.c1);
    const int H = k.hout, Wd = k.wout;
    SEEDRL_TRY(conv_bwd(c, k.r11, N, H, Wd, c1, IN_RELU, gA, c1, nullptr, gB));
    SEEDRL_TRY(conv_bwd(c, k.r10, N, H, Wd, o0, IN_RELU, gB, o0, gA, gC));
    SEEDRL_TRY(conv_bwd(c, k.r01, N, H, Wd, c0, IN_RELU, gC, c0, nullptr, gB));
    SEEDRL_TRY(conv_bwd(c, k.r00, N, H, Wd, p, IN_RELU, gB, p, gC, gA));
    SEEDRL_TRY(maxpool3s2_backward(N, k.hin, k.win, k.c, gA, W<uint8_t>(ws, b.idx), gF, st));
    const void* x = s == 0 ? (const void*)obs : (const void*)W<float>(ws, pl.st[s - 1].o1);
    if (s == 0 && generic_first(n))
      SEEDRL_TRY(conv3x3_u8_wgrad(first_c(n), N, k.hin, k.win, obs, gF, c.G(k.conv.w), c.G(k.conv.b),
                                  W<float>(ws, pl.partial), conv3x3_wgrad_partial_bytes(), st));
    else
      SEEDRL_TRY(conv_bwd(c, k.conv, N, k.hin, k.win, x, s == 0 ? IN_U8 : IN_F32, gF, nullptr,
                          nullptr, s == 0 ? nullptr : gA));
  }
  return SEEDRL_OK;
}

static int planes_conv_bwd(Call& c, const ConvLayer& l, int N, int H, int Wd, const void* x, const void* dy,
                           const void* dmask, const void* dres, void* dx) {
  SEEDRL_TRY(wgradp(l.cin, l.cout, N, H, Wd, x, dy, c.G(l.w), c.G(l.b), c.ex.err, &c.wb, c.ex.st));
  if (dx) {
    g_conv_cat = PC_CONV_DGRAD;
    const int rc = planes_conv(c, l.cout, l.cin, N, H, Wd, dy, c.P(l.w), 1, nullptr, dmask, dres,
                               dx, nullptr, nullptr);
    g_conv_cat = PC_CONV_FWD;
    SEEDRL_TRY(rc);
  }
  return SEEDRL_OK;
}

static int torso_backward_planes(Call& c, const uint8_t* obs) {
  const seedrl_net* n = c.n; const Plan& pl = c.pl; void* ws = c.ws; cudaStream_t st = c.ex.st;
  const int N = pl.N;
  void* g1 = W<void>(ws, pl.gP1); void* g2 = W<void>(ws, pl.gP2); void* g3 = W<void>(ws, pl.gP3);
  void* gfp = W<void>(ws, pl.gFP); float* gF = W<float>(ws, pl.gFull);
  {
    const Stack& k = n->stacks.back();
    SEEDRL_TRY(to_planes(N, k.hout, k.wout, k.c, 0, W<float>(ws, pl.gA), g1, st));
  }
  for (int s = (int)n->stacks.size() - 1; s >= 0; --s) {
    const Stack& k = n->stacks[s];
    const StackBufs& b = pl.st[s];
    const int H = k.hout, Wd = k.wout;
    const void* prelu = W<void>(ws, b.prelu); const void* c0r = W<void>(ws, b.c0r);
    const void* o0relu = W<void>(ws, b.o0relu); const void* c1r = W<void>(ws, b.c1r);
    SEEDRL_TRY(planes_conv_bwd(c, k.r11, N, H, Wd, c1r, g1, c1r, nullptr, g2));
    SEEDRL_TRY(planes_conv_bwd(c, k.r10, N, H, Wd, o0relu, g2, o0relu, g1, g3));
    SEEDRL_TRY(planes_conv_bwd(c, k.r01, N, H, Wd, c0r, g3, c0r, nullptr, g2));
    SEEDRL_TRY(planes_conv_bwd(c, k.r00, N, H, Wd, prelu, g2, prelu, g3, g1));
    if (s == 0 && first_wgrad_pooled_supported(first_c(n), k.c, k.hin, k.win) && !g_first_dense) {
      SEEDRL_TRY(first_wgrad_pooled(N, k.hin, k.win, first_c(n), obs, g1, W<uint8_t>(ws, b.idx), c.G(k.conv.w),
                                    c.G(k.conv.b), &c.wb, st));
    } else if (s == 0 && generic_first(n)) {
      return set_error(SEEDRL_ERR_INVALID_ARGUMENT,
                       "the dense first-layer path takes 3- or 4-channel frames; switch it off for these frames");
    } else if (s == 0) {
      SEEDRL_TRY(poolp_backward(N, k.hin, k.win, k.c, g1, W<uint8_t>(ws, b.idx), nullptr, gF, st));
      SEEDRL_TRY(conv_bwd(c, k.conv, N, k.hin, k.win, obs, IN_U8, gF, nullptr, nullptr, nullptr));
    } else {
      SEEDRL_TRY(poolp_backward(N, k.hin, k.win, k.c, g1, W<uint8_t>(ws, b.idx), gfp, nullptr, st));
      SEEDRL_TRY(planes_conv_bwd(c, k.conv, N, k.hin, k.win, W<void>(ws, pl.st[s - 1].o1p), gfp, nullptr,
                                 nullptr, g1));
    }
  }
  return SEEDRL_OK;
}

static int torso_backward_shallow(Call& c, const uint8_t* obs) {
  const seedrl_net* n = c.n; const Plan& pl = c.pl; void* ws = c.ws; cudaStream_t st = c.ex.st;
  const int N = pl.N;
  float* gA = W<float>(ws, pl.gA); float* gB = W<float>(ws, pl.gB);
  const float* a1 = W<float>(ws, pl.sh_a1);
  if (n->conv_mode >= 1 && n->cfg.obs_c % 4 == 0) {
    const StridedConv &l0 = n->sh[0], &l1 = n->sh[1];
    float* col1 = W<float>(ws, pl.sh_col1);
    SEEDRL_TRY(l1.wgrad(c.ex, N, false, a1, col1, gA, c.G(n->sh_w[1]), 32, c.G(n->sh_b[1])));
    SEEDRL_TRY(l1.dgrad(c.ex, N, gA, c.P(n->sh_w[1]), col1, a1, gB));
    return l0.wgrad(c.ex, N, true, obs, W<float>(ws, pl.sh_col0), gB, c.G(n->sh_w[0]), 16, c.G(n->sh_b[0]));
  }
  SEEDRL_TRY(convgen_wgrad(N, n->sh[0].hout, n->sh[0].wout, 16, 32, 4, 2, 0, a1, gA, c.G(n->sh_w[1]),
                           c.G(n->sh_b[1]), W<float>(ws, pl.partial),
                           conv3x3_wgrad_partial_bytes(), st));
  SEEDRL_TRY(convgen_dgrad(N, n->sh[0].hout, n->sh[0].wout, 16, 32, 4, 2, gA, c.P(n->sh_w[1]), a1, gB, st));
  SEEDRL_TRY(convgen_wgrad(N, n->cfg.obs_h, n->cfg.obs_w, n->cfg.obs_c, 16, 8, 4, 1, obs, gB,
                           c.G(n->sh_w[0]), c.G(n->sh_b[0]), W<float>(ws, pl.partial),
                           conv3x3_wgrad_partial_bytes(), st));
  return SEEDRL_OK;
}

static int net_backward(const seedrl_net* n, const float* prm, int T1, int B, const uint8_t* done,
                        const uint8_t* observation, const float* dlogits, const float* dbaseline, float* grd,
                        void* ws, size_t ws_bytes, cudaEvent_t head_ready, cudaStream_t st) {
  SEEDRL_CHECK_ARG(n && prm && done && observation && dlogits && dbaseline && grd && ws,
                   "null pointer");
  const Plan pl = make_plan(n, T1, B);
  SEEDRL_CHECK_ARG(ws_bytes >= pl.total, "workspace too small");
  Call c(n, pl, prm, grd, ws, st);
  c.head_ready = head_ready;
  const int N = pl.N, A = n->cfg.num_actions, CI = n->core_in;
  float* xc = W<float>(ws, pl.xc); float* z = W<float>(ws, pl.z);
  float* hp = W<float>(ws, pl.hp); float* cs = W<float>(ws, pl.cs);
  float* hs = W<float>(ws, pl.hs); float* c0buf = W<float>(ws, pl.c0buf);
  float* dhs = W<float>(ws, pl.dhs); float* dz = W<float>(ws, pl.dz);
  float* dhrec = W<float>(ws, pl.dhrec); float* dd = W<float>(ws, pl.dd);
  float* dcb[2] = {W<float>(ws, pl.dc0), W<float>(ws, pl.dc1)};
  SEEDRL_CUDA(cudaMemsetAsync(grd, 0, n->params.arena_floats * sizeof(float), st));

  GemmEpi e = epi_none();
  SEEDRL_TRY(c.ex.gemm(true, false, kHidden, A, N, hs, kHidden, dlogits, A, c.G(n->p_pol_w), A, e));
  SEEDRL_TRY(c.ex.colsum(N, A, dlogits, A, c.G(n->p_pol_b)));
  SEEDRL_TRY(c.ex.gemm(true, false, kHidden, 1, N, hs, kHidden, dbaseline, 1, c.G(n->p_base_w), 1, e));
  SEEDRL_TRY(c.ex.colsum(N, 1, dbaseline, 1, c.G(n->p_base_b)));
  SEEDRL_TRY(c.ex.gemm(false, true, N, kHidden, A, dlogits, A, c.P(n->p_pol_w), A, dhs, kHidden, e));
  GemmEpi eacc = epi_none();
  eacc.accumulate = 1;
  SEEDRL_TRY(c.ex.gemm(false, true, N, kHidden, 1, dbaseline, 1, c.P(n->p_base_w), 1, dhs, kHidden,
                   eacc));
  SEEDRL_TRY(lstm_recurrence_backward(n->lstm_mode, c.ex, kHidden, T1, B, c.P(n->p_core_u), done, z, cs, c0buf, dhs,
                                      dz, dhrec, dcb, W<unsigned int>(ws, pl.counter)));
  SEEDRL_TRY(c.ex.gemm(true, false, kHidden, 4 * kHidden, N, hp, kHidden, dz, 4 * kHidden,
                   c.G(n->p_core_u), 4 * kHidden, e));
  SEEDRL_TRY(c.ex.gemm(true, false, CI, 4 * kHidden, N, xc, CI, dz, 4 * kHidden, c.G(n->p_core_w),
                   4 * kHidden, e));
  SEEDRL_TRY(c.ex.colsum(N, 4 * kHidden, dz, 4 * kHidden, c.G(n->p_core_b)));
  GemmEpi em = epi_none();
  em.mask = xc; em.ldm = CI;
  SEEDRL_TRY(c.ex.gemm(false, true, N, kHidden, 4 * kHidden, dz, 4 * kHidden, c.P(n->p_core_w),
                   4 * kHidden, dd, kHidden, em));
  const float* flat_src = n->cfg.net == SEEDRL_NET_DEEP ? W<float>(ws, pl.st.back().o1)
                                                        : W<float>(ws, pl.sh_a2);
  GemmEpi ea = epi_none();
  ea.a_relu = n->cfg.net == SEEDRL_NET_DEEP ? 1 : 0;
  SEEDRL_TRY(c.ex.gemm(true, false, n->flat, kHidden, N, flat_src, n->flat, dd, kHidden,
                   c.G(n->p_dense_w), kHidden, ea));
  SEEDRL_TRY(c.ex.colsum(N, kHidden, dd, kHidden, c.G(n->p_dense_b)));
  if (c.head_ready) SEEDRL_CUDA(cudaEventRecord(c.head_ready, st));
  GemmEpi ef = epi_none();
  ef.mask = flat_src; ef.ldm = n->flat;
  SEEDRL_TRY(c.ex.gemm(false, true, N, n->flat, kHidden, dd, kHidden, c.P(n->p_dense_w), kHidden,
                   W<float>(ws, pl.gA), n->flat, ef));
  if (n->cfg.net == SEEDRL_NET_DEEP) {
    c.wb = WgradBatch{W<float>(ws, pl.partial_all), kPartialAllBytes / sizeof(float), 0, 0, {}};
    SEEDRL_TRY(pad_first_layer(c, &observation));
    SEEDRL_TRY(pack_all_weights(c, 1));
    SEEDRL_TRY(n->conv_mode == 3 ? torso_backward_planes(c, observation) : torso_backward_deep(c, observation));
    SEEDRL_TRY(wgrad_reduce_batch(&c.wb, st));
    if (c.dw0_pad) {
      unpad_dw0_kernel<<<ceil_div(9 * 3 * 16, 128), 128, 0, st>>>(16, c.dw0_pad,
                                                                   grd + n->params.offset(n->stacks[0].conv.w));
      count_launch(PC_MISC, st);
    }
    return SEEDRL_OK;
  }
  return torso_backward_shallow(c, observation);
}

extern "C" int seedrl_net_backward(const seedrl_net* n, const float* prm, int T1, int B,
                                   const int64_t* prev_actions, const float* reward,
                                   const uint8_t* done, const uint8_t* observation,
                                   const float* dlogits, const float* dbaseline, float* grd,
                                   void* ws, size_t ws_bytes, seedrl_stream_t stream) {
  (void)prev_actions; (void)reward;
  return net_backward(n, prm, T1, B, done, observation, dlogits, dbaseline, grd, ws, ws_bytes, nullptr,
                      (cudaStream_t)stream);
}

extern "C" int seedrl_net_backward_overlap(const seedrl_net* n, const float* prm, int T1, int B,
                                           const int64_t* prev_actions, const float* reward, const uint8_t* done,
                                           const uint8_t* observation, const float* dlogits, const float* dbaseline,
                                           float* grd, void* ws, size_t ws_bytes, void* head_ready_event,
                                           seedrl_stream_t stream) {
  (void)prev_actions; (void)reward;
  return net_backward(n, prm, T1, B, done, observation, dlogits, dbaseline, grd, ws, ws_bytes,
                      (cudaEvent_t)head_ready_event, (cudaStream_t)stream);
}
extern "C" size_t seedrl_net_grad_split(const seedrl_net* n) {
  if (!n) return 0;
  const int first_conv = n->cfg.net == SEEDRL_NET_DEEP ? n->stacks[0].conv.w : n->sh_w[0];
  return n->params.offset(first_conv);
}

extern "C" int seedrl_debug_conv3x3(int cin, int cout, int in_mode, int N, int H, int W,
                                    const void* in, const float* w, const float* bias,
                                    const float* mask, const float* res, float* out,
                                    seedrl_stream_t stream) {
  return conv3x3_forward(cin, cout, in_mode, N, H, W, in, w, bias, mask, res, out,
                         (cudaStream_t)stream);
}
extern "C" int seedrl_debug_conv3x3_flip(int cin, int cout, const float* w, float* wt,
                                         seedrl_stream_t stream) {
  return conv3x3_flip_weights(cin, cout, w, wt, (cudaStream_t)stream);
}
extern "C" size_t seedrl_debug_wgrad_partial_bytes(void) { return conv3x3_wgrad_partial_bytes(); }
extern "C" int seedrl_debug_conv3x3_wgrad(int cin, int cout, int in_mode, int N, int H, int W,
                                          const void* x, const float* dy, float* dw, float* db,
                                          float* partial, size_t partial_bytes,
                                          seedrl_stream_t stream) {
  return conv3x3_wgrad(cin, cout, in_mode, N, H, W, x, dy, dw, db, partial, partial_bytes,
                       (cudaStream_t)stream);
}
extern "C" int seedrl_debug_maxpool(int backward, int N, int H, int W, int C, const float* x_or_dy,
                                    float* y_or_dx, uint8_t* idx, seedrl_stream_t stream) {
  if (backward) return maxpool3s2_backward(N, H, W, C, x_or_dy, idx, y_or_dx, (cudaStream_t)stream);
  return maxpool3s2_forward(N, H, W, C, x_or_dy, y_or_dx, idx, (cudaStream_t)stream);
}
extern "C" int seedrl_debug_gemm_tc(int ta, int tb, int split, int M, int N, int K, const float* A, int lda,
                                    const float* B, int ldb, float* C, int ldc, const float* bias,
                                    const float* mask, int ldm, int relu, int accumulate, int a_relu,
                                    float* ws, size_t ws_bytes, int* error_flag, seedrl_stream_t stream) {
  SEEDRL_CHECK_ARG(M >= 1 && N >= 1 && K >= 1 && A && B && C, "bad arguments");
  GemmEpi e{bias, mask, ldm, relu, accumulate, a_relu};
  return gemm_tc(ta != 0, tb != 0, split, M, N, K, A, lda, B, ldb, C, ldc, e, ws, ws_bytes, error_flag,
                 (cudaStream_t)stream);
}

extern "C" int seedrl_debug_sgemm(int ta, int tb, int M, int N, int K, const float* A, int lda,
                                  const float* B, int ldb, float* C, int ldc, const float* bias,
                                  const float* mask, int ldm, int relu, int accumulate, int a_relu,
                                  seedrl_stream_t stream) {
  GemmEpi e{bias, mask, ldm, relu, accumulate, a_relu};
  return sgemm(ta != 0, tb != 0, M, N, K, A, lda, B, ldb, C, ldc, e, (cudaStream_t)stream);
}

extern "C" int seedrl_debug_set_gemm_gather(int on) {
  gemm_tc_set_gather(on);
  return SEEDRL_OK;
}

extern "C" int seedrl_debug_colsum(int M, int N, const float* X, int ld, float* out, float* ws, size_t ws_bytes,
                                   seedrl_stream_t stream) {
  SEEDRL_CHECK_ARG(M >= 1 && N >= 1 && X && out && ld >= N, "bad arguments");
  return colsum(M, N, X, ld, out, (cudaStream_t)stream, ws, ws_bytes);
}

extern "C" int seedrl_debug_conv_pixels(int N, int H, int W, int which, int start, int count, int* out) {
  SEEDRL_CHECK_ARG(N >= 1 && H >= 1 && W >= 1 && start >= 0 && count >= 0 && out, "bad arguments");
  const ConvGeom g = make_geom(N, H, W);
  for (int i = 0; i < count; ++i) out[i] = which ? out_pixel(g, start + i) : in_pixel(g, start + i);
  return SEEDRL_OK;
}

extern "C" int seedrl_debug_set_wgrad_chunk(int kc) {
  SEEDRL_CHECK_ARG(kc == 128 || kc == 256 || kc == 512, "chunk must be 128, 256 or 512");
  conv3x3_wgrad_tc_set_chunk(kc);
  return SEEDRL_OK;
}

extern "C" int seedrl_debug_conv3x3_wgrad_tc(int cin, int cout, int in_mode, int split, int N, int H, int W,
                                             const void* x, const float* dy, float* dw, float* db,
                                             float* partial, size_t partial_bytes, int* error_flag,
                                             seedrl_stream_t stream) {
  SEEDRL_CHECK_ARG(conv3x3_wgrad_tc_supported(cin, cout, in_mode), "unsupported (cin,cout,mode)");
  return conv3x3_wgrad_tc(cin, cout, in_mode, split, N, H, W, x, dy, dw, db, partial, partial_bytes,
                          error_flag, nullptr, (cudaStream_t)stream);
}
extern "C" int seedrl_debug_conv0pool(int N, int H, int W, const uint8_t* frames, const float* w, const float* bias,
                                      void* praw, void* prelu, uint8_t* idx, int* err, seedrl_stream_t stream) {
  SEEDRL_CHECK_ARG(frames && w && bias && praw && prelu && idx && err, "null pointer");
  SEEDRL_CHECK_ARG(conv0pool_supported(4, 16, H, W), "unsupported frame size");
  return conv0pool_forward(N, H, W, 4, frames, w, bias, praw, prelu, idx, err, (cudaStream_t)stream);
}
extern "C" int seedrl_debug_conv0pool_c(int N, int H, int W, int C, const uint8_t* frames, const float* w,
                                        const float* bias, void* praw, void* prelu, uint8_t* idx, int* err,
                                        seedrl_stream_t stream) {
  SEEDRL_CHECK_ARG(frames && w && bias && praw && prelu && idx && err, "null pointer");
  SEEDRL_CHECK_ARG(N >= 1 && conv0pool_supported(C, 16, H, W), "unsupported frame shape");
  return conv0pool_forward(N, H, W, C, frames, w, bias, praw, prelu, idx, err, (cudaStream_t)stream);
}
extern "C" int seedrl_debug_first_wgrad_pooled_c(int N, int H, int W, int C, const uint8_t* frames,
                                                 const void* g_planes, const uint8_t* idx, float* dw, float* db,
                                                 float* partial, size_t partial_bytes, seedrl_stream_t stream) {
  SEEDRL_CHECK_ARG(frames && g_planes && idx && dw && db && partial, "null pointer");
  SEEDRL_CHECK_ARG(N >= 1 && first_wgrad_pooled_supported(C, 16, H, W), "unsupported frame shape");
  WgradBatch wb{partial, partial_bytes / sizeof(float), 0, 0, {}};
  SEEDRL_TRY(first_wgrad_pooled(N, H, W, C, frames, g_planes, idx, dw, db, &wb, (cudaStream_t)stream));
  return wgrad_reduce_batch(&wb, (cudaStream_t)stream);
}
extern "C" int seedrl_debug_set_first_layer_dense(int on) {
  g_first_dense = on ? 1 : 0;
  return SEEDRL_OK;
}
extern "C" int seedrl_debug_set_gemm_bk(int bk) {
  gemm_tc_set_bk(bk);
  return SEEDRL_OK;
}
extern "C" int seedrl_debug_set_conv_tile(int mt) {
  SEEDRL_CHECK_ARG(mt == 128 || mt == 256 || mt == 512, "tile must be 128, 256 or 512");
  conv3x3_tc_set_tile(mt);
  return SEEDRL_OK;
}

extern "C" int seedrl_debug_conv3x3_tc(int cin, int cout, int in_mode, int split, int N, int H, int W,
                                       const void* in, const float* w, const float* bias,
                                       const float* mask, const float* res, float* out, int flip,
                                       int variant, void* wq_scratch, int* error_flag,
                                       seedrl_stream_t stream) {
  SEEDRL_CHECK_ARG(conv3x3_tc_supported(cin, cout, in_mode), "unsupported (cin,cout,mode)");
  SEEDRL_TRY(conv3x3_tc_pack_weights(cin, cout, flip, split, w, wq_scratch, (cudaStream_t)stream));
  return conv3x3_tc_forward(cin, cout, in_mode, split, N, H, W, in, wq_scratch, bias, mask, res, out,
                            variant, error_flag, (cudaStream_t)stream);
}

extern "C" size_t seedrl_debug_planes_bytes(int N, int H, int W, int C) {
  if (N < 1 || H < 1 || W < 1 || C < 8 || C % 8) return 0;
  return planes_bytes(N, H, W, C);
}
extern "C" int seedrl_debug_to_planes(int N, int H, int W, int C, int relu, const float* x, void* out,
                                      seedrl_stream_t stream) {
  SEEDRL_CHECK_ARG(N >= 1 && H >= 1 && W >= 1 && C >= 8 && C % 8 == 0 && x && out, "bad arguments");
  return to_planes(N, H, W, C, relu, x, out, (cudaStream_t)stream);
}
extern "C" int seedrl_debug_from_planes(int N, int H, int W, int C, const void* in, float* y,
                                        seedrl_stream_t stream) {
  SEEDRL_CHECK_ARG(N >= 1 && H >= 1 && W >= 1 && C >= 8 && C % 8 == 0 && in && y, "bad arguments");
  return from_planes(N, H, W, C, in, y, (cudaStream_t)stream);
}
extern "C" int seedrl_debug_convp(int cin, int cout, int N, int H, int W, const void* in, const float* w,
                                  const float* bias, const void* mask, const void* res, int flip,
                                  void* out_raw, void* out_relu, float* out_nhwc, void* wq_scratch,
                                  int* error_flag, seedrl_stream_t stream) {
  SEEDRL_CHECK_ARG(convp_supported(cin, cout) && in && w && wq_scratch, "unsupported (cin,cout) or null pointer");
  SEEDRL_TRY(conv3x3_tc_pack_weights(cin, cout, flip, 2, w, wq_scratch, (cudaStream_t)stream));
  PlaneConv c;
  c.N = N; c.H = H; c.W = W; c.in = in; c.wq = wq_scratch; c.bias = bias; c.mask = mask; c.res = res;
  c.out_raw = out_raw; c.out_relu = out_relu; c.out_nhwc = out_nhwc; c.err = error_flag;
  return convp_forward(cin, cout, c, (cudaStream_t)stream);
}
extern "C" int seedrl_debug_wgradp(int cin, int cout, int N, int H, int W, const void* x, const void* dy,
                                   float* dw, float* db, float* partial, size_t partial_bytes,
                                   int* error_flag, seedrl_stream_t stream) {
  SEEDRL_CHECK_ARG(x && dy && dw && db && partial, "null pointer");
  WgradBatch wb{partial, partial_bytes / sizeof(float), 0, 0, {}};
  SEEDRL_TRY(wgradp(cin, cout, N, H, W, x, dy, dw, db, error_flag, &wb, (cudaStream_t)stream));
  return wgrad_reduce_batch(&wb, (cudaStream_t)stream);
}
extern "C" int seedrl_debug_poolp(int backward, int N, int H, int W, int C, const void* in, void* out_raw,
                                  void* out_relu, float* out_nhwc, uint8_t* idx, seedrl_stream_t stream) {
  SEEDRL_CHECK_ARG(N >= 1 && H >= 1 && W >= 1 && C >= 8 && C % 8 == 0 && in && idx, "bad arguments");
  if (backward) return poolp_backward(N, H, W, C, in, idx, out_raw, out_nhwc, (cudaStream_t)stream);
  SEEDRL_CHECK_ARG(out_raw && out_relu, "null pointer");
  return poolp_forward(N, H, W, C, reinterpret_cast<const float*>(in), out_raw, out_relu, idx,
                       (cudaStream_t)stream);
}
```

Baseline: 168,300.

## Fuse conv dgrad into planes wgrad kernel sharing TMA-loaded dy stages

For 16-channel-input residual convs, the backward pass now runs weight-gradient and data-gradient in one kernel. Two extra warpgroups consume the same TMA-staged dy tiles with wgmma and the packed flipped weights, applying the mask and residual epilogue, so dy is read from global memory once and one launch is saved per conv. It also factors the forward MMA and epilogue into shared device functions and disables Python cyclic GC during CUDA graph capture. In exchange the kernel needs more threads and shared memory, the stage pipeline now covers the dgrad chunk count, and the wgrad descriptor offset changes, which is a correctness risk.

```diff
diff --git a/include/seedrl_b200.h b/include/seedrl_b200.h
--- a/include/seedrl_b200.h
+++ b/include/seedrl_b200.h
@@ -292,6 +292,10 @@
 int seedrl_debug_wgradp(int cin, int cout, int N, int H, int W, const void* x, const void* dy,
                         float* dw, float* db, float* partial, size_t partial_bytes,
                         int* error_flag, seedrl_stream_t stream);
+int seedrl_debug_convp_bwd(int cin, int cout, int N, int H, int W, const void* x, const void* dy,
+                           const float* w, int mask, const void* res, void* dx, float* dw, float* db,
+                           void* wq_scratch, float* partial, size_t partial_bytes, int* error_flag,
+                           seedrl_stream_t stream);
 int seedrl_debug_poolp(int backward, int N, int H, int W, int C, const void* in, void* out_raw,
                        void* out_relu, float* out_nhwc, uint8_t* idx, seedrl_stream_t stream);
 
diff --git a/seed_rl_b200/_lib.py b/seed_rl_b200/_lib.py
--- a/seed_rl_b200/_lib.py
+++ b/seed_rl_b200/_lib.py
@@ -147,6 +147,8 @@
     'seedrl_debug_from_planes': (c_int, [c_int, c_int, c_int, c_int, P, P, P]),
     'seedrl_debug_convp': (c_int, [c_int, c_int, c_int, c_int, c_int, P, P, P, P, P, c_int, P, P, P, P, P, P]),
     'seedrl_debug_wgradp': (c_int, [c_int, c_int, c_int, c_int, c_int, P, P, P, P, P, c_size_t, P, P]),
+    'seedrl_debug_convp_bwd': (c_int, [c_int, c_int, c_int, c_int, c_int, P, P, P, c_int, P, P, P, P, P, P,
+                                       c_size_t, P, P]),
     'seedrl_debug_poolp': (c_int, [c_int, c_int, c_int, c_int, c_int, P, P, P, P, P, P]),
     'seedrl_debug_conv3x3': (c_int, [c_int, c_int, c_int, c_int, c_int, c_int, P, P, P, P, P, P, P]),
     'seedrl_debug_conv3x3_flip': (c_int, [c_int, c_int, P, P, P]),
diff --git a/seed_rl_b200/common/inference_host.py b/seed_rl_b200/common/inference_host.py
--- a/seed_rl_b200/common/inference_host.py
+++ b/seed_rl_b200/common/inference_host.py
@@ -1,3 +1,7 @@
+import contextlib
+import gc
+import threading
+
 from absl import logging
 import numpy as np
 import torch
@@ -5,6 +9,27 @@
 from seed_rl_b200 import _lib
 from seed_rl_b200.common import utils
 from seed_rl_b200.grpc import ops as grpc
+
+_capture_lock = threading.Lock()
+_captures = 0
+_gc_was_enabled = False
+
+
+@contextlib.contextmanager
+def _no_cyclic_gc():
+  global _captures, _gc_was_enabled
+  with _capture_lock:
+    if _captures == 0:
+      _gc_was_enabled = gc.isenabled()
+      gc.disable()
+    _captures += 1
+  try:
+    yield
+  finally:
+    with _capture_lock:
+      _captures -= 1
+      if _captures == 0 and _gc_was_enabled:
+        gc.enable()
 
 
 class InferenceHostBase(object):
@@ -117,7 +142,7 @@
       t.copy_(sv)
     self.stream.synchronize()
     g = torch.cuda.CUDAGraph()
-    with torch.cuda.graph(g, stream=self.stream, capture_error_mode='thread_local'):
+    with _no_cyclic_gc(), torch.cuda.graph(g, stream=self.stream, capture_error_mode='thread_local'):
       self._g_prev_states, self._g_out = self._device_step(self._g_ids, self._g_env, self._g_counter)
     self._graph = g
 
diff --git a/seed_rl_b200/csrc/conv_planes.cu b/seed_rl_b200/csrc/conv_planes.cu
--- a/seed_rl_b200/csrc/conv_planes.cu
+++ b/seed_rl_b200/csrc/conv_planes.cu
@@ -120,10 +120,95 @@
   }
 }
 
+template <int CIN, int COUT>
+__device__ __forceinline__ void convp_block_mma(float (&acc)[COUT], uint64_t da0, uint64_t db0, uint64_t lo_off,
+                                                uint64_t slab_off, int m, int PW) {
+  constexpr int NS = CIN / 16;
+#pragma unroll
+  for (int i = 0; i < COUT; ++i) acc[i] = 0.f;
+  wgmma_fence_acc<COUT>(acc);
+  wgmma_fence();
+#pragma unroll
+  for (int tap = 0; tap < 9; ++tap) {
+    const uint64_t off = (uint64_t)(m * 64 + (tap / 3) * PW + (tap % 3));
+#pragma unroll
+    for (int sl = 0; sl < NS; ++sl) {
+      const uint64_t da = da0 + off + (uint64_t)sl * slab_off;
+      const uint64_t db = db0 + (uint64_t)((tap * NS + sl) * (COUT * 64 / 16));
+      Wgmma<2 * COUT>::template mma<0, 0>(acc, da, db, 1u);
+      Wgmma<COUT>::template mma<0, 0>(acc, da + lo_off, db, 1u);
+    }
+  }
+  wgmma_commit();
+}
+
+template <int COUT>
+__device__ __forceinline__ void convp_epilogue(const float (&acc)[COUT], int q, int pix, int sp, bool in_store,
+                                               size_t plane_u, const float* s_bias, bool mask,
+                                               const uint4 (&mk)[COUT / 16], bool res, const uint4 (&rh)[COUT / 16],
+                                               const uint4 (&rl)[COUT / 16], uint4* out_raw, uint4* out_relu,
+                                               float* out_nhwc) {
+  constexpr int GO = COUT / 8;
+#pragma unroll
+  for (int k = 0; k < GO / 2; ++k) {
+    const int go = (q >> 1) + 2 * k;
+    float2 t[4];
+#pragma unroll
+    for (int u = 0; u < 4; ++u) {
+      const int j = 2 * k + (u >> 1), h = u & 1;
+      t[u] = make_float2(acc[4 * j + 2 * h] + acc[4 * (j + GO) + 2 * h],
+                         acc[4 * j + 2 * h + 1] + acc[4 * (j + GO) + 2 * h + 1]);
+    }
+    quad_transpose(t, q);
+    float x[8];
+#pragma unroll
+    for (int e = 0; e < 4; ++e) {
+      x[2 * e] = t[e].x + s_bias[go * 8 + 2 * e];
+      x[2 * e + 1] = t[e].y + s_bias[go * 8 + 2 * e + 1];
+    }
+    if (pix >= 0 && mask) {
+      const uint32_t mw[4] = {mk[k].x, mk[k].y, mk[k].z, mk[k].w};
+#pragma unroll
+      for (int e = 0; e < 4; ++e) {
+        x[2 * e] = bf16lo(mw[e]) > 0.f ? x[2 * e] : 0.f;
+        x[2 * e + 1] = bf16hi(mw[e]) > 0.f ? x[2 * e + 1] : 0.f;
+      }
+    }
+    if (pix >= 0 && res) {
+      const uint32_t hw[4] = {rh[k].x, rh[k].y, rh[k].z, rh[k].w};
+      const uint32_t lw[4] = {rl[k].x, rl[k].y, rl[k].z, rl[k].w};
+#pragma unroll
+      for (int e = 0; e < 4; ++e) {
+        x[2 * e] += bf16lo(hw[e]) + bf16lo(lw[e]);
+        x[2 * e + 1] += bf16hi(hw[e]) + bf16hi(lw[e]);
+      }
+    }
+    if (pix < 0) {
+#pragma unroll
+      for (int e = 0; e < 8; ++e) x[e] = 0.f;
+    }
+    const float4 xa = make_float4(x[0], x[1], x[2], x[3]), xb = make_float4(x[4], x[5], x[6], x[7]);
+    if (out_raw && in_store) {
+      out_raw[(size_t)go * plane_u + sp] = pack8_bf16(xa, xb);
+      out_raw[(size_t)(GO + go) * plane_u + sp] = pack8_bf16(bf16_resid4(xa), bf16_resid4(xb));
+    }
+    if (out_relu && in_store) {
+      const float4 ra = make_float4(fmaxf(xa.x, 0.f), fmaxf(xa.y, 0.f), fmaxf(xa.z, 0.f), fmaxf(xa.w, 0.f));
+      const float4 rb = make_float4(fmaxf(xb.x, 0.f), fmaxf(xb.y, 0.f), fmaxf(xb.z, 0.f), fmaxf(xb.w, 0.f));
+      out_relu[(size_t)go * plane_u + sp] = pack8_bf16(ra, rb);
+      out_relu[(size_t)(GO + go) * plane_u + sp] = pack8_bf16(bf16_resid4(ra), bf16_resid4(rb));
+    }
+    if (out_nhwc && pix >= 0) {
+      float4* o = reinterpret_cast<float4*>(out_nhwc + (size_t)pix * COUT + go * 8);
+      o[0] = xa; o[1] = xb;
+    }
+  }
+}
+
 template <int CIN, int COUT, int NSUB>
 __global__ void __launch_bounds__(kCpThreads, 1)
 convp_kernel(const __grid_constant__ CUtensorMap tm_in, const ConvpArgs a) {
-  constexpr int G = CIN / 8, GO = COUT / 8, NS = CIN / 16;
+  constexpr int G = CIN / 8, GO = COUT / 8;
   constexpr int MT = NSUB * kCpM;
   constexpr int NBLK = 2 * NSUB;
   extern __shared__ __align__(128) uint8_t smem_raw[];
@@ -191,22 +276,7 @@
 #pragma unroll 1
       for (int m = m0; m < NBLK; m += kCpWarpgroups) {
         float acc[COUT];
-#pragma unroll
-        for (int i = 0; i < COUT; ++i) acc[i] = 0.f;
-        wgmma_fence_acc<COUT>(acc);
-        wgmma_fence();
-#pragma unroll
-        for (int tap = 0; tap < 9; ++tap) {
-          const uint64_t off = (uint64_t)(m * 64 + (tap / 3) * PW + (tap % 3));
-#pragma unroll
-          for (int sl = 0; sl < NS; ++sl) {
-            const uint64_t da = da0 + off + (uint64_t)sl * slab_off;
-            const uint64_t db = db0 + (uint64_t)((tap * NS + sl) * (COUT * 64 / 16));
-            Wgmma<2 * COUT>::template mma<0, 0>(acc, da, db, 1u);
-            Wgmma<COUT>::template mma<0, 0>(acc, da + lo_off, db, 1u);
-          }
-        }
-        wgmma_commit();
+        convp_block_mma<CIN, COUT>(acc, da0, db0, lo_off, slab_off, m, PW);
         const int p = tile * MT + m * 64 + row;
         const int sp = p + PW + 1;
         const int pix = out_pixel(a.g, p);
@@ -225,61 +295,8 @@
         wgmma_wait<0>();
         wgmma_fence_acc<COUT>(acc);
         if (m + kCpWarpgroups >= NBLK && lane == 0) mbar_arrive(s_empty + s);
-        const bool in_store = sp < a.Lp;
-#pragma unroll
-        for (int k = 0; k < GO / 2; ++k) {
-          const int go = (q >> 1) + 2 * k;
-          float2 t[4];
-#pragma unroll
-          for (int u = 0; u < 4; ++u) {
-            const int j = 2 * k + (u >> 1), h = u & 1;
-            t[u] = make_float2(acc[4 * j + 2 * h] + acc[4 * (j + GO) + 2 * h],
-                               acc[4 * j + 2 * h + 1] + acc[4 * (j + GO) + 2 * h + 1]);
-          }
-          quad_transpose(t, q);
-          float x[8];
-#pragma unroll
-          for (int e = 0; e < 4; ++e) {
-            x[2 * e] = t[e].x + s_bias[go * 8 + 2 * e];
-            x[2 * e + 1] = t[e].y + s_bias[go * 8 + 2 * e + 1];
-          }
-          if (pix >= 0 && a.mask) {
-            const uint32_t mw[4] = {mk[k].x, mk[k].y, mk[k].z, mk[k].w};
-#pragma unroll
-            for (int e = 0; e < 4; ++e) {
-              x[2 * e] = bf16lo(mw[e]) > 0.f ? x[2 * e] : 0.f;
-              x[2 * e + 1] = bf16hi(mw[e]) > 0.f ? x[2 * e + 1] : 0.f;
-            }
-          }
-          if (pix >= 0 && a.res) {
-            const uint32_t hw[4] = {rh[k].x, rh[k].y, rh[k].z, rh[k].w};
-            const uint32_t lw[4] = {rl[k].x, rl[k].y, rl[k].z, rl[k].w};
-#pragma unroll
-            for (int e = 0; e < 4; ++e) {
-              x[2 * e] += bf16lo(hw[e]) + bf16lo(lw[e]);
-              x[2 * e + 1] += bf16hi(hw[e]) + bf16hi(lw[e]);
-            }
-          }
-          if (pix < 0) {
-#pragma unroll
-            for (int e = 0; e < 8; ++e) x[e] = 0.f;
-          }
-          const float4 xa = make_float4(x[0], x[1], x[2], x[3]), xb = make_float4(x[4], x[5], x[6], x[7]);
-          if (a.out_raw && in_store) {
-            a.out_raw[(size_t)go * plane_u + sp] = pack8_bf16(xa, xb);
-            a.out_raw[(size_t)(GO + go) * plane_u + sp] = pack8_bf16(bf16_resid4(xa), bf16_resid4(xb));
-          }
-          if (a.out_relu && in_store) {
-            const float4 ra = make_float4(fmaxf(xa.x, 0.f), fmaxf(xa.y, 0.f), fmaxf(xa.z, 0.f), fmaxf(xa.w, 0.f));
-            const float4 rb = make_float4(fmaxf(xb.x, 0.f), fmaxf(xb.y, 0.f), fmaxf(xb.z, 0.f), fmaxf(xb.w, 0.f));
-            a.out_relu[(size_t)go * plane_u + sp] = pack8_bf16(ra, rb);
-            a.out_relu[(size_t)(GO + go) * plane_u + sp] = pack8_bf16(bf16_resid4(ra), bf16_resid4(rb));
-          }
-          if (a.out_nhwc && pix >= 0) {
-            float4* o = reinterpret_cast<float4*>(a.out_nhwc + (size_t)pix * COUT + go * 8);
-            o[0] = xa; o[1] = xb;
-          }
-        }
+        convp_epilogue<COUT>(acc, q, pix, sp, sp < a.Lp, plane_u, s_bias, a.mask != nullptr, mk, a.res != nullptr,
+                             rh, rl, a.out_raw, a.out_relu, a.out_nhwc);
       }
     }
   }
@@ -353,21 +370,33 @@
   int chunk;
   float* partial;
   int* err;
+  ConvGeom g;
+  int Lp;
+  int dchunks;
+  const uint4* wq;
+  int mask;
+  const uint4* res;
+  uint4* dx;
 };
 
 constexpr int kWpMaxStages = 6;
 constexpr int kWpHaloRow = 8;
 __host__ __device__ constexpr int wgradp_mtiles(int CP) { return 3 * CP + 1 <= 64 ? 1 : 2; }
 __host__ __device__ constexpr int wgradp_khsplit(int CP) { return CP == 16 ? 3 : 1; }
-__host__ __device__ constexpr int wgradp_threads(int CP) { return 128 * wgradp_mtiles(CP) * wgradp_khsplit(CP) + 32; }
+__host__ __device__ constexpr int wgradp_dgrad_wgs(bool dgrad) { return dgrad ? 2 : 0; }
+__host__ __device__ constexpr int wgradp_threads(int CP, bool dgrad) {
+  return 128 * (wgradp_mtiles(CP) * wgradp_khsplit(CP) + wgradp_dgrad_wgs(dgrad)) + 32;
+}
+bool convp_bwd_supported(int cin, int cout) { return cin == 16 && (cout == 16 || cout == 32); }
 
 struct WgradMaps { CUtensorMap x, x_halo, dy, dy_halo; };
 
-template <int CP, int COUT, int KC>
-__global__ void __launch_bounds__(wgradp_threads(CP), 1)
+template <int CP, int COUT, int KC, bool DGRAD>
+__global__ void __launch_bounds__(wgradp_threads(CP, DGRAD), 1)
 wgradp_kernel(const __grid_constant__ WgradMaps tm, const WgradpArgs a) {
   constexpr int G = CP / 8, GO = COUT / 8;
   constexpr int MT = wgradp_mtiles(CP), KSPL = wgradp_khsplit(CP), NCW = MT * KSPL;
+  constexpr int ND = wgradp_dgrad_wgs(DGRAD);
   constexpr int NKH = 3 / KSPL;
   constexpr int NW = 9 * CP * COUT + COUT;
   constexpr uint32_t Px = (KC + kWpHaloRow) * 16;
@@ -379,20 +408,29 @@
   uint64_t* s_full = reinterpret_cast<uint64_t*>(smem_raw);
   uint64_t* s_empty = s_full + kWpMaxStages;
   uint8_t* s_stage = smem_raw + 128;
+  uint4* s_w = reinterpret_cast<uint4*>(s_stage + (size_t)nb * stage_bytes);
+  float* s_zero = reinterpret_cast<float*>(s_w + 2 * 9 * COUT * CP / 8);
   const int tid = threadIdx.x, warp = tid >> 5, lane = tid & 31;
 
+  if (DGRAD) {
+    for (int i = tid; i < 2 * 9 * COUT * CP / 8; i += (int)blockDim.x) s_w[i] = __ldg(a.wq + i);
+    if (tid < CP) s_zero[tid] = 0.f;
+  }
   if (tid == 0) {
-    for (int i = 0; i < kWpMaxStages; ++i) { mbar_init(s_full + i, 1); mbar_init(s_empty + i, 4 * NCW); }
+    for (int i = 0; i < kWpMaxStages; ++i) { mbar_init(s_full + i, 1); mbar_init(s_empty + i, 4 * (NCW + ND)); }
     asm volatile("fence.mbarrier_init.release.cluster;" ::: "memory");
   }
+  if (DGRAD) asm volatile("fence.proxy.async.shared::cta;" ::: "memory");
   __syncthreads();
 
+  const int nall = DGRAD ? a.dchunks : a.nchunks;
   const int my_chunks = ((int)blockIdx.x < a.nchunks) ? (a.nchunks - 1 - (int)blockIdx.x) / (int)gridDim.x + 1 : 0;
+  const int my_all = ((int)blockIdx.x < nall) ? (nall - 1 - (int)blockIdx.x) / (int)gridDim.x + 1 : 0;
   bool timed_out = false;
 
-  if (warp == 4 * NCW) {
+  if (warp == 4 * (NCW + ND)) {
     if (elect_one()) {
-      for (int it = 0; it < my_chunks; ++it) {
+      for (int it = 0; it < my_all; ++it) {
         const int s = it % nb;
         if (it >= nb && !mbar_wait_bounded(s_empty + s, (uint32_t)(((it / nb) - 1) & 1))) { timed_out = true; break; }
         const int j0 = ((int)blockIdx.x + it * (int)gridDim.x) * KC;
@@ -410,7 +448,7 @@
       }
     }
     __syncwarp();
-  } else {
+  } else if (warp < 4 * NCW) {
     const int cw = warp >> 2, mt = cw % MT, kh0 = (cw / MT) * NKH;
     const int mg0 = 8 * mt + 2 * (warp & 3);
     const int mg = mg0 + ((lane >> 3) & 1);
@@ -430,7 +468,7 @@
       if (!mbar_wait_bounded(s_full + s, (uint32_t)((it / nb) & 1))) { timed_out = true; break; }
       const uint32_t sb = smem_u32(s_stage + (size_t)s * stage_bytes);
       const uint32_t xb = sb + a_off;
-      const uint32_t db = desc_lo + ((sb + x_bytes) >> 4) + (uint32_t)((2 - kh0) * PW);
+      const uint32_t db = desc_lo + ((sb + x_bytes) >> 4) + (uint32_t)((2 - kh0) * PW + 1);
       uint32_t ah[2][4], al[2][4];
 #pragma unroll
       for (int ks = 0; ks < KC / 16; ++ks) {
@@ -453,6 +491,11 @@
       wgmma_wait<0>();
       if (lane == 0) mbar_arrive(s_empty + s);
     }
+    for (int it = my_chunks; it < my_all && !timed_out; ++it) {
+      const int s = it % nb;
+      if (!mbar_wait_bounded(s_full + s, (uint32_t)((it / nb) & 1))) { timed_out = true; break; }
+      if (lane == 0) mbar_arrive(s_empty + s);
+    }
     wgmma_fence_acc<NKH * COUT>(&acc[0][0]);
     float* dst = a.partial + (size_t)blockIdx.x * NW;
 #pragma unroll
@@ -474,69 +517,147 @@
         }
       }
     }
+  } else if constexpr (DGRAD) {
+    constexpr int NBLK = KC / 64;
+    const int dw = (warp >> 2) - NCW;
+    const size_t plane_u = (size_t)a.Lp;
+    if (blockIdx.x == 0) {
+      const uint4 z = make_uint4(0u, 0u, 0u, 0u);
+      for (int i = tid - 128 * NCW; i < (PW + 1) * 2 * G; i += 128 * ND) {
+        const int pl = i / (PW + 1), s = i - pl * (PW + 1);
+        a.dx[(size_t)pl * plane_u + s] = z;
+      }
+    }
+    const int q = lane & 3;
+    const int row = 16 * (warp & 3) + (lane >> 2) + 8 * (q & 1);
+    const uint64_t db0 = gmma_desc(smem_u32(s_w), (uint32_t)(2 * G) * 128u, 128u);
+    const uint64_t lo_off = (uint64_t)((GO * Pd) >> 4), slab_off = (uint64_t)((2 * Pd) >> 4);
+    for (int it = 0; it < my_all; ++it) {
+      const int s = it % nb;
+      const int j0 = ((int)blockIdx.x + it * (int)gridDim.x) * KC;
+      if (!mbar_wait_bounded(s_full + s, (uint32_t)((it / nb) & 1))) { timed_out = true; break; }
+      const int m0 = (dw - it * NBLK) & (ND - 1);
+      if (m0 >= NBLK && lane == 0) mbar_arrive(s_empty + s);
+      const uint8_t* xs = s_stage + (size_t)s * stage_bytes;
+      const uint64_t da0 = gmma_desc(smem_u32(xs + x_bytes), Pd, 128u);
+#pragma unroll 1
+      for (int m = m0; m < NBLK; m += ND) {
+        float acc[CP];
+        convp_block_mma<COUT, CP>(acc, da0, db0, lo_off, slab_off, m, PW);
+        const int p = j0 + m * 64 + row;
+        const int sp = p + PW + 1;
+        const int pix = out_pixel(a.g, p);
+        uint4 mk[G / 2], rh[G / 2], rl[G / 2];
+        if (pix >= 0) {
+#pragma unroll
+          for (int k = 0; k < G / 2; ++k) {
+            const int go = (q >> 1) + 2 * k;
+            if (a.mask) mk[k] = reinterpret_cast<const uint4*>(xs + go * Px)[m * 64 + row + 1];
+            if (a.res) {
+              rh[k] = __ldg(a.res + (size_t)go * plane_u + sp);
+              rl[k] = __ldg(a.res + (size_t)(G + go) * plane_u + sp);
+            }
+          }
+        }
+        wgmma_wait<0>();
+        wgmma_fence_acc<CP>(acc);
+        if (m + ND >= NBLK && lane == 0) mbar_arrive(s_empty + s);
+        convp_epilogue<CP>(acc, q, pix, sp, sp < a.Lp, plane_u, s_zero, a.mask != 0, mk, a.res != nullptr, rh, rl,
+                           a.dx, nullptr, nullptr);
+      }
+    }
   }
   if (timed_out && a.err) atomicExch(a.err, 1);
 }
 
-template <int CP, int COUT, int KC>
+struct DgradOperands { const void* wq; int mask; const void* res; void* dx; };
+
+template <int CP, int COUT, int KC, bool DGRAD>
 static int launch_wgradp(int N, int H, int W, const void* x, const void* dy, float* dw, float* db, int* err,
-                         WgradBatch* batch, cudaStream_t st) {
+                         WgradBatch* batch, const DgradOperands* d, cudaStream_t st) {
   const ConvGeom g = make_geom(N, H, W);
   const long long Lp = planes_positions(N, H, W);
   constexpr int G = CP / 8, GO = COUT / 8;
+  if (Lp + KC + 4 * g.PW >= (1LL << 31))
+    return set_error(SEEDRL_ERR_INVALID_ARGUMENT, "wgradp: batch too large for 32-bit positions");
   const int CH = planes_chunk() < KC ? planes_chunk() : KC;
   if (KC % CH) return kPlanesTryNext;
-  const int T = (2 * g.PW + kWpHaloRow - 1) / kWpHaloRow * kWpHaloRow;
+  const int T = (2 * g.PW + 2 + kWpHaloRow - 1) / kWpHaloRow * kWpHaloRow;
   const size_t stage = (size_t)2 * G * (KC + kWpHaloRow) * 16 + (size_t)2 * GO * (KC + T) * 16;
   int nb = kWpMaxStages;
   while (nb > 1 && 128 + nb * stage > 227 * 1024) --nb;
   if (nb < 2) return kPlanesTryNext;
-  const size_t smem = 128 + nb * stage;
+  const size_t extra = DGRAD ? (size_t)2 * 9 * CP * COUT * 2 + CP * 4 : 0;
+  while (nb > 1 && 128 + nb * stage + extra > 227 * 1024) --nb;
+  if (nb < 2) return set_error(SEEDRL_ERR_INVALID_ARGUMENT, "conv backward: image too wide");
+  const size_t smem = 128 + nb * stage + extra;
   WgradMaps tm;
   SEEDRL_TRY(make_plane_map(&tm.x, x, Lp, 2 * G, g.PW, CH, KC / CH, 1));
   SEEDRL_TRY(make_plane_map(&tm.x_halo, x, Lp, 2 * G, g.PW, kWpHaloRow, 1, 1));
-  SEEDRL_TRY(make_plane_map(&tm.dy, dy, Lp, 2 * GO, 1, CH, KC / CH, 1));
-  SEEDRL_TRY(make_plane_map(&tm.dy_halo, dy, Lp, 2 * GO, 1, kWpHaloRow, T / kWpHaloRow, 1));
+  SEEDRL_TRY(make_plane_map(&tm.dy, dy, Lp, 2 * GO, 0, CH, KC / CH, 1));
+  SEEDRL_TRY(make_plane_map(&tm.dy_halo, dy, Lp, 2 * GO, 0, kWpHaloRow, T / kWpHaloRow, 1));
   static bool attr = false;
   if (!attr) {
-    SEEDRL_CUDA(cudaFuncSetAttribute(wgradp_kernel<CP, COUT, KC>, cudaFuncAttributeMaxDynamicSharedMemorySize,
-                                     227 * 1024));
+    SEEDRL_CUDA(cudaFuncSetAttribute(wgradp_kernel<CP, COUT, KC, DGRAD>,
+                                     cudaFuncAttributeMaxDynamicSharedMemorySize, 227 * 1024));
     attr = true;
   }
   static const bool dbg = getenv("SEEDRL_DEBUG_LAUNCH") != nullptr;
-  if (dbg) fprintf(stderr, "wgradp<%d,%d,%d> CH=%d T=%d nb=%d stage=%zu smem=%zu\n", CP, COUT, KC, CH, T, nb, stage, smem);
+  if (dbg)
+    fprintf(stderr, "wgradp<%d,%d,%d,%d> CH=%d T=%d nb=%d stage=%zu smem=%zu\n", CP, COUT, KC, (int)DGRAD, CH, T, nb,
+            stage, smem);
   constexpr int NW = 9 * CP * COUT + COUT;
-  WgradpArgs a;
+  WgradpArgs a = {};
   a.PW = g.PW; a.T = T; a.nb = nb; a.err = err; a.chunk = CH;
   a.nchunks = (int)((g.Q + g.PW + KC - 1) / KC);
+  if (DGRAD) {
+    a.g = g; a.Lp = (int)Lp;
+    a.dchunks = (int)((Lp - g.PW - 1 + KC - 1) / KC);
+    a.wq = reinterpret_cast<const uint4*>(d->wq); a.mask = d->mask;
+    a.res = reinterpret_cast<const uint4*>(d->res); a.dx = reinterpret_cast<uint4*>(d->dx);
+  }
   const int grid = a.nchunks < kNumSMs ? a.nchunks : kNumSMs;
   if (!batch || batch->n >= kMaxReduceJobs || batch->used + (size_t)grid * NW > batch->cap_floats)
     return set_error(SEEDRL_ERR_INVALID_ARGUMENT, "wgradp: partial buffer too small");
   a.partial = batch->buf + batch->used;
   batch->used += (size_t)grid * NW;
-  wgradp_kernel<CP, COUT, KC><<<grid, wgradp_threads(CP), smem, st>>>(tm, a);
+  wgradp_kernel<CP, COUT, KC, DGRAD><<<grid, wgradp_threads(CP, DGRAD), smem, st>>>(tm, a);
   count_launch(PC_CONV_WGRAD, st);
   SEEDRL_CHECK_LAUNCH();
   batch->jobs[batch->n++] = ReduceJob{a.partial, dw, db, grid, 9 * CP * COUT, COUT};
   return SEEDRL_OK;
 }
 
+template <bool DGRAD>
+static int wgradp_any(int cin, int cout, int N, int H, int W, const void* x, const void* dy, float* dw, float* db,
+                      int* err, WgradBatch* batch, const DgradOperands* d, cudaStream_t st) {
+#define SEEDRL_WP_CASE(CI, CO_, KC0)                                                                             \
+  if (cin == CI && cout == CO_) {                                                                                \
+    int rc = kPlanesTryNext;                                                                                     \
+    if constexpr (KC0 >= 256) rc = launch_wgradp<CI, CO_, 256, DGRAD>(N, H, W, x, dy, dw, db, err, batch, d, st); \
+    if (rc == kPlanesTryNext) rc = launch_wgradp<CI, CO_, 128, DGRAD>(N, H, W, x, dy, dw, db, err, batch, d, st); \
+    if (rc == kPlanesTryNext) rc = launch_wgradp<CI, CO_, 64, DGRAD>(N, H, W, x, dy, dw, db, err, batch, d, st);  \
+    if (rc == kPlanesTryNext) return set_error(SEEDRL_ERR_INVALID_ARGUMENT, "wgradp: does not fit");             \
+    return rc;                                                                                                   \
+  }
+  SEEDRL_WP_CASE(16, 16, 256)
+  SEEDRL_WP_CASE(16, 32, 128)
+  if constexpr (!DGRAD) SEEDRL_WP_CASE(32, 32, 128)
+#undef SEEDRL_WP_CASE
+  return set_error(SEEDRL_ERR_INVALID_ARGUMENT, "wgradp: unsupported (cin,cout)");
+}
+
 int wgradp(int cin, int cout, int N, int H, int W, const void* x, const void* dy, float* dw, float* db,
            int* err, WgradBatch* batch, cudaStream_t st) {
-#define SEEDRL_WP_CASE(CI, CO_, KC0)                                                                        \
-  if (cin == CI && cout == CO_) {                                                                           \
-    int rc = kPlanesTryNext;                                                                                \
-    if constexpr (KC0 >= 256) rc = launch_wgradp<CI, CO_, 256>(N, H, W, x, dy, dw, db, err, batch, st);     \
-    if (rc == kPlanesTryNext) rc = launch_wgradp<CI, CO_, 128>(N, H, W, x, dy, dw, db, err, batch, st);     \
-    if (rc == kPlanesTryNext) rc = launch_wgradp<CI, CO_, 64>(N, H, W, x, dy, dw, db, err, batch, st);      \
-    if (rc == kPlanesTryNext) return set_error(SEEDRL_ERR_INVALID_ARGUMENT, "wgradp: does not fit");        \
-    return rc;                                                                                              \
-  }
-  SEEDRL_WP_CASE(16, 16, 256)
-  SEEDRL_WP_CASE(16, 32, 128)
-  SEEDRL_WP_CASE(32, 32, 128)
-#undef SEEDRL_WP_CASE
-  return set_error(SEEDRL_ERR_INVALID_ARGUMENT, "wgradp: unsupported (cin,cout)");
+  return wgradp_any<false>(cin, cout, N, H, W, x, dy, dw, db, err, batch, nullptr, st);
+}
+
+int convp_bwd(int cin, int cout, int N, int H, int W, const void* x, const void* dy, const void* wq, int mask,
+              const void* res, void* dx, float* dw, float* db, int* err, WgradBatch* batch, cudaStream_t st) {
+  if (!dx || !convp_bwd_supported(cin, cout))
+    return set_error(SEEDRL_ERR_INVALID_ARGUMENT, "convp_bwd: null dx or unsupported (cin,cout)");
+  const DgradOperands d{wq, mask, res, dx};
+  return wgradp_any<true>(cin, cout, N, H, W, x, dy, dw, db, err, batch, &d, st);
 }
 
 __global__ void to_planes_kernel(ConvGeom g, int Lp, int G, int relu, const float* __restrict__ x,
diff --git a/seed_rl_b200/csrc/kernels.h b/seed_rl_b200/csrc/kernels.h
--- a/seed_rl_b200/csrc/kernels.h
+++ b/seed_rl_b200/csrc/kernels.h
@@ -95,6 +95,9 @@
 int convp_forward(int cin, int cout, const PlaneConv& c, cudaStream_t st);
 int wgradp(int cin, int cout, int N, int H, int W, const void* x, const void* dy, float* dw, float* db,
            int* err, WgradBatch* batch, cudaStream_t st);
+bool convp_bwd_supported(int cin, int cout);
+int convp_bwd(int cin, int cout, int N, int H, int W, const void* x, const void* dy, const void* wq, int mask,
+              const void* res, void* dx, float* dw, float* db, int* err, WgradBatch* batch, cudaStream_t st);
 int to_planes(int N, int H, int W, int C, int relu, const float* x, void* out, cudaStream_t st);
 int from_planes(int N, int H, int W, int C, const void* in, float* y, cudaStream_t st);
 int poolp_forward(int N, int H, int W, int C, const float* x, void* out_raw, void* out_relu, uint8_t* idx,
diff --git a/seed_rl_b200/csrc/net.cu b/seed_rl_b200/csrc/net.cu
--- a/seed_rl_b200/csrc/net.cu
+++ b/seed_rl_b200/csrc/net.cu
@@ -598,16 +598,19 @@
 }
 
 static int planes_conv_bwd(Call& c, const ConvLayer& l, int N, int H, int Wd, const void* x, const void* dy,
-                           const void* dmask, const void* dres, void* dx) {
+                           int mask, const void* dres, void* dx) {
+  if (convp_bwd_supported(l.cin, l.cout)) {
+    const void* wq;
+    SEEDRL_TRY(packed_weights(c, l.cout, l.cin, c.P(l.w), 1, 2, &wq));
+    return convp_bwd(l.cin, l.cout, N, H, Wd, x, dy, wq, mask, dres, dx, c.G(l.w), c.G(l.b), c.ex.err, &c.wb,
+                     c.ex.st);
+  }
   SEEDRL_TRY(wgradp(l.cin, l.cout, N, H, Wd, x, dy, c.G(l.w), c.G(l.b), c.ex.err, &c.wb, c.ex.st));
-  if (dx) {
-    g_conv_cat = PC_CONV_DGRAD;
-    const int rc = planes_conv(c, l.cout, l.cin, N, H, Wd, dy, c.P(l.w), 1, nullptr, dmask, dres,
-                               dx, nullptr, nullptr);
-    g_conv_cat = PC_CONV_FWD;
-    SEEDRL_TRY(rc);
-  }
-  return SEEDRL_OK;
+  g_conv_cat = PC_CONV_DGRAD;
+  const int rc = planes_conv(c, l.cout, l.cin, N, H, Wd, dy, c.P(l.w), 1, nullptr, mask ? x : nullptr, dres,
+                             dx, nullptr, nullptr);
+  g_conv_cat = PC_CONV_FWD;
+  return rc;
 }
 
 static int torso_backward_planes(Call& c, const uint8_t* obs) {
@@ -625,10 +628,10 @@
     const int H = k.hout, Wd = k.wout;
     const void* prelu = W<void>(ws, b.prelu); const void* c0r = W<void>(ws, b.c0r);
     const void* o0relu = W<void>(ws, b.o0relu); const void* c1r = W<void>(ws, b.c1r);
-    SEEDRL_TRY(planes_conv_bwd(c, k.r11, N, H, Wd, c1r, g1, c1r, nullptr, g2));
-    SEEDRL_TRY(planes_conv_bwd(c, k.r10, N, H, Wd, o0relu, g2, o0relu, g1, g3));
-    SEEDRL_TRY(planes_conv_bwd(c, k.r01, N, H, Wd, c0r, g3, c0r, nullptr, g2));
-    SEEDRL_TRY(planes_conv_bwd(c, k.r00, N, H, Wd, prelu, g2, prelu, g3, g1));
+    SEEDRL_TRY(planes_conv_bwd(c, k.r11, N, H, Wd, c1r, g1, 1, nullptr, g2));
+    SEEDRL_TRY(planes_conv_bwd(c, k.r10, N, H, Wd, o0relu, g2, 1, g1, g3));
+    SEEDRL_TRY(planes_conv_bwd(c, k.r01, N, H, Wd, c0r, g3, 1, nullptr, g2));
+    SEEDRL_TRY(planes_conv_bwd(c, k.r00, N, H, Wd, prelu, g2, 1, g3, g1));
     if (s == 0 && first_wgrad_pooled_supported(first_c(n), k.c, k.hin, k.win) && !g_first_dense) {
       SEEDRL_TRY(first_wgrad_pooled(N, k.hin, k.win, first_c(n), obs, g1, W<uint8_t>(ws, b.idx), c.G(k.conv.w),
                                     c.G(k.conv.b), &c.wb, st));
@@ -640,7 +643,7 @@
       SEEDRL_TRY(conv_bwd(c, k.conv, N, k.hin, k.win, obs, IN_U8, gF, nullptr, nullptr, nullptr));
     } else {
       SEEDRL_TRY(poolp_backward(N, k.hin, k.win, k.c, g1, W<uint8_t>(ws, b.idx), gfp, nullptr, st));
-      SEEDRL_TRY(planes_conv_bwd(c, k.conv, N, k.hin, k.win, W<void>(ws, pl.st[s - 1].o1p), gfp, nullptr,
+      SEEDRL_TRY(planes_conv_bwd(c, k.conv, N, k.hin, k.win, W<void>(ws, pl.st[s - 1].o1p), gfp, 0,
                                  nullptr, g1));
     }
   }
@@ -915,6 +918,18 @@
   SEEDRL_TRY(wgradp(cin, cout, N, H, W, x, dy, dw, db, error_flag, &wb, (cudaStream_t)stream));
   return wgrad_reduce_batch(&wb, (cudaStream_t)stream);
 }
+extern "C" int seedrl_debug_convp_bwd(int cin, int cout, int N, int H, int W, const void* x, const void* dy,
+                                     const float* w, int mask, const void* res, void* dx, float* dw, float* db,
+                                     void* wq_scratch, float* partial, size_t partial_bytes, int* error_flag,
+                                     seedrl_stream_t stream) {
+  SEEDRL_CHECK_ARG(x && dy && w && dx && dw && db && wq_scratch && partial, "null pointer");
+  SEEDRL_CHECK_ARG(convp_supported(cout, cin), "unsupported (cin,cout)");
+  SEEDRL_TRY(conv3x3_tc_pack_weights(cout, cin, 1, 2, w, wq_scratch, (cudaStream_t)stream));
+  WgradBatch wb{partial, partial_bytes / sizeof(float), 0, 0, {}};
+  SEEDRL_TRY(convp_bwd(cin, cout, N, H, W, x, dy, wq_scratch, mask, res, dx, dw, db, error_flag, &wb,
+                       (cudaStream_t)stream));
+  return wgrad_reduce_batch(&wb, (cudaStream_t)stream);
+}
 extern "C" int seedrl_debug_poolp(int backward, int N, int H, int W, int C, const void* in, void* out_raw,
                                   void* out_relu, float* out_nhwc, uint8_t* idx, seedrl_stream_t stream) {
   SEEDRL_CHECK_ARG(N >= 1 && H >= 1 && W >= 1 && C >= 8 && C % 8 == 0 && in && idx, "bad arguments");
```

Measured after the change: 176,000 (median of 6 runs). 4.6% higher.
